# FanmingL/Recurrent-Offpolicy-RL

Hardware: AMD Instinct MI355X
Metric: env-steps/sec trained (higher is better)
Workload: dtype f32; 1 GPU; smamba_s32_c16_b2_nln SAC-REDQ update, B=64/GPU, T=1024, D=256 (configs[1]; N=8: configs[3]); row_length=1043, obs=17, act=6, critic=efc-8, global_rows=64, parallelism=dp1

## Files before the change

include/resel_hip.h:

```cpp
#ifndef RESEL_HIP_H
#define RESEL_HIP_H

#include <stddef.h>
#include <stdint.h>

#ifdef __cplusplus
extern "C" {
#endif

#define RESEL_OK 0
#define RESEL_EINVAL (-1)
#define RESEL_ELAUNCH (-2)

typedef void* resel_stream_t;

int resel_abi_version(void);
const char* resel_build_info(void);

enum {
    RESEL_PROF_SSCAN_FWD = 0, RESEL_PROF_SSCAN_BWD = 1, RESEL_PROF_ATTN_FWD = 2, RESEL_PROF_ATTN_DQ = 3, RESEL_PROF_ATTN_DKV = 4,
    RESEL_PROF_LINREC_REAL_FWD = 5, RESEL_PROF_LINREC_REAL_BWD = 6, RESEL_PROF_LINREC_COMPLEX_FWD = 7, RESEL_PROF_LINREC_COMPLEX_BWD = 8,
    RESEL_PROF_GRU_FWD = 9, RESEL_PROF_GRU_BWD = 10, RESEL_PROF_CONV_FWD = 11, RESEL_PROF_CONV_BWD = 12, RESEL_PROF_GEMM = 13,
    RESEL_PROF_SSCAN_FWD_LOCAL = 14, RESEL_PROF_SSCAN_BWD_LOCAL = 15,
    RESEL_PROF_NSLOTS = 16
// ... 10 lines not shown
                             const float* D, const float* delta_bias, const float* start,
                             float* out, int64_t ld_out, float* ckpt, float* last_state, void* workspace,
                             int B, int L, int Di, int N, int delta_softplus, int time_segments,
                             void* amax_out, unsigned amax_epoch, resel_stream_t stream);

size_t resel_selective_scan_bwd_workspace_bytes(int B, int L, int Di, int N, int time_segments);
int resel_selective_scan_bwd(const float* u, int64_t ld_u, const float* delta, int64_t ld_delta,
                             const float* z, int64_t ld_z, const float* A,
                             const float* Bm, int64_t ld_b, const float* Cm, int64_t ld_c,
                             const float* D, const float* delta_bias, const float* start,
                             const float* dout, int64_t ld_dout, const float* ckpt,
                             float* du, int64_t ld_du, float* ddelta, int64_t ld_ddelta, float* dz, int64_t ld_dz,
                             float* dBm, int64_t ld_db, float* dCm, int64_t ld_dc,
                             float* dA, float* dD, float* ddelta_bias, void* workspace,
                             int B, int L, int Di, int N, int delta_softplus, int time_segments,
                             void* amax_dz, void* amax_ddelta, unsigned amax_epoch, resel_stream_t stream);

int resel_causal_conv1d_fwd(const float* x, int64_t ld_x, const float* w, const float* bias, const float* mask,
                            float* y, int64_t ld_y, int B, int L, int Di, int K, int silu, void* amax_y, unsigned amax_epoch,
                            resel_stream_t stream);
size_t resel_causal_conv1d_bwd_workspace_bytes(int B, int L, int Di, int K);
int resel_causal_conv1d_bwd(const float* x, int64_t ld_x, const float* w, const float* bias, const float* mask,
                            const float* dy, int64_t ld_dy, float* dx, int64_t ld_dx, float* dw, float* dbias,
                            void* workspace, int B, int L, int Di, int K, int silu, void* amax_dx, unsigned amax_epoch,
                            resel_stream_t stream);
int resel_causal_conv1d_bwd2(const float* x, int64_t ld_x, const float* w, const float* bias, const float* mask,
                             const float* dy, int64_t ld_dy, const float* dy2, int64_t ld_dy2, float* dx, int64_t ld_dx,
                             float* dw, float* dbias, void* workspace, int B, int L, int Di, int K, int silu,
                             void* amax_dx, unsigned amax_epoch, resel_stream_t stream);

int resel_add_layernorm_fwd(const float* x, const float* residual, const float* w, const float* b,
                            float* y, float* res_out, float* stats, int M, int C, float eps, int rms, int act,
                            void* amax_y, unsigned amax_epoch, resel_stream_t stream);
size_t resel_add_layernorm_bwd_workspace_bytes(int M, int C);
int resel_add_layernorm_bwd(const float* dy, const float* dres_in, const float* res, const float* w, const float* b,
                            const float* stats, float* dx, float* dw, float* db, void* workspace,
                            int M, int C, int rms, int has_bias, int act, void* amax_dx, unsigned amax_epoch, resel_stream_t stream);

int resel_linrec_real_fwd(const float* v, const float* f, int64_t ld_u, const float* start, const float* h0, float* h,
                          int B, int L, int C, int fuse_act, void* amax_h, unsigned amax_epoch, resel_stream_t stream);
int resel_linrec_real_bwd(const float* v, const float* f, int64_t ld_u, const float* start, const float* h0, const float* h,
                          const float* dh, float* dv, float* df, int64_t ld_du, int B, int L, int C, int fuse_act,
                          void* amax_du, unsigned amax_epoch, resel_stream_t stream);
int resel_linrec_complex_fwd(const float* vr, const float* vi, int64_t ld_u, const float* lam_re, const float* lam_im,
                             const float* gamma, const float* start, const float* h0r, const float* h0i,
                             float* hr, float* hi, int B, int L, int C, void* amax_h, unsigned amax_epoch, resel_stream_t stream);
size_t resel_linrec_complex_bwd_workspace_bytes(int B, int L, int C);
int resel_linrec_complex_bwd(const float* vr, const float* vi, int64_t ld_u, const float* lam_re, const float* lam_im,
                             const float* gamma, const float* start, const float* h0r, const float* h0i,
                             const float* hr, const float* hi, const float* dhr, const float* dhi,
                             float* dvr, float* dvi, int64_t ld_du, float* dlam_re, float* dlam_im, float* dgamma,
                             void* workspace, int B, int L, int C, resel_stream_t stream);

int resel_lru_params_fwd(const float* params_log, float* out, int C, resel_stream_t stream);
int resel_lru_params_bwd(const float* params_log, const float* dout, float* dparams_log, int C, resel_stream_t stream);

size_t resel_gru_workspace_bytes(int B, int L, int H);
int resel_gru_seq_fwd(const float* gi, const float* w_hh, const float* b_hh, const float* h0,
                      float* h_all, float* gates, void* workspace, int B, int L, int H, resel_stream_t stream);
int resel_gru_seq_bwd(const float* w_hh, const float* h0, const float* h_all, const float* gates,
                      const float* dh_all, float* dgi, float* dgh, void* workspace,
                      int B, int L, int H, resel_stream_t stream);

size_t resel_attn_varlen_fwd_workspace_bytes(int S, int max_seqlen);
int resel_attn_varlen_fwd(const uint16_t* qkv, const int32_t* cu_seqlens, const float* slopes, uint16_t* out, float* lse,
                          void* workspace, int T, int S, int H, int hd, int max_seqlen, float scale,
                          float p_drop, uint64_t seed, uint64_t offset, resel_stream_t stream);
size_t resel_attn_varlen_bwd_workspace_bytes(int T, int S, int H, int hd, int max_seqlen);
int resel_attn_varlen_bwd(const uint16_t* qkv, const int32_t* cu_seqlens, const float* slopes, const uint16_t* out,
                          const float* lse, const uint16_t* dout, uint16_t* dqkv, void* workspace,
                          int T, int S, int H, int hd, int max_seqlen, float scale,
                          float p_drop, uint64_t seed, uint64_t offset, resel_stream_t stream);

int resel_dropout(const float* x, float* y, int64_t n, float p_drop, uint64_t seed, uint64_t offset, resel_stream_t stream);
int resel_dropout_offset_base(const void* base);
int resel_gelu_dropout_fwd(const float* x, float* y, int64_t n, float p_drop, uint64_t seed, uint64_t offset,
                           void* amax_y, unsigned amax_epoch, resel_stream_t stream);
int resel_gelu_dropout_bwd(const float* x, const float* dy, float* dx, int64_t n, float p_drop, uint64_t seed, uint64_t offset,
                           void* amax_dx, unsigned amax_epoch, resel_stream_t stream);

int resel_tanh_gaussian_fwd(const float* out2, const float* noise, float* action_mean, float* action_sample,
                            float* logp, int M, int A, resel_stream_t stream);
int resel_tanh_gaussian_bwd(const float* out2, const float* noise, const float* d_sample, const float* d_logp,
                            float* d_out2, int M, int A, resel_stream_t stream);

int resel_sac_target(const float* q, const int32_t* subset, int m, const float* next_logp, const float* log_alpha,
                     const float* reward, const float* done, const float* mask, float gamma, float* guard,
                     float* target, float* stats, void* workspace, int E, int M, resel_stream_t stream);
int resel_sac_target_phase(int phase, const float* q, const int32_t* subset, int m, const float* next_logp, const float* log_alpha,
                           const float* reward, const float* done, const float* mask, float gamma, float* guard,
                           float* target, float* stats, float* extrema, void* workspace, int E, int M, resel_stream_t stream);
int resel_sac_target_local(const float* q, const int32_t* subset, int m, const float* next_logp, const float* log_alpha,
                           const float* reward, const float* done, const float* mask, float gamma, const float* guard,
                           float* target, float* stats, float* extrema, void* workspace, int E, int M, resel_stream_t stream);
int resel_guard_apply_slots(const float* slots, int world, float* guard, resel_stream_t stream);
size_t resel_sac_target_workspace_bytes(int M);

size_t resel_masked_loss_workspace_bytes(void);
int resel_q_loss_fwd(const float* q, const float* y, const float* mask, float* out2, void* workspace, int E, int M, resel_stream_t stream);
int resel_q_loss_bwd(const float* q, const float* y, const float* mask, const float* g, float* dq, int E, int M, resel_stream_t stream);
int resel_actor_loss_fwd(const float* logp, const float* q, const float* mask, const float* log_alpha, float* out2, void* workspace,
                         int E, int M, int use_logp, int reduce_min, resel_stream_t stream);
int resel_actor_loss_bwd(const float* q, const float* mask, const float* log_alpha, const float* g, float* dlogp, float* dq,
                         int E, int M, int use_logp, int reduce_min, resel_stream_t stream);

int resel_soft_update(float* target, const float* online, float tau, int64_t n, resel_stream_t stream);
int resel_adamw_flat(float* p, const float* g, float* m, float* v, int64_t n, const int64_t* seg_end,
                     const float* seg_lr, const float* seg_wd, int nseg, float beta1, float beta2, float eps,
                     int step, const float* grad_scale, resel_stream_t stream);
int resel_adamw_flat_dev(float* p, const float* g, float* m, float* v, int64_t n, const int64_t* seg_end,
                         const float* seg_lr, const float* seg_wd, int nseg, float beta1, float beta2, float eps,
                         const float* bias_corrections, const float* grad_scale, resel_stream_t stream);
size_t resel_sumsq_workspace_bytes(int64_t n);
int resel_sumsq(const float* x, int64_t n, float* out, void* workspace, resel_stream_t stream);

int resel_bias_act_fwd(float* y, const float* bias, int64_t rows, int C, int64_t rows_per_seg, int act, resel_stream_t stream);
size_t resel_bias_act_bwd_workspace_bytes(int64_t rows, int C, int64_t rows_per_seg);
int resel_bias_act_bwd(const float* g, int64_t ldg, const float* a, int64_t lda, float* gy, float* dbias, void* workspace, int64_t rows, int C,
                       int64_t rows_per_seg, int act, void* amax_gy, unsigned amax_epoch, resel_stream_t stream);

int resel_ensemble_head_fwd(float* y, const float* b2, const float* w3, const float* b3, float* q, int64_t rows, int H,
                            int64_t rows_per_seg, resel_stream_t stream);
size_t resel_ensemble_head_bwd_workspace_bytes(int64_t rows, int H, int64_t rows_per_seg);
int resel_ensemble_head_bwd(const float* gq, const float* a, const float* w3, float* gy, float* db2, float* dw3, void* workspace,
                            int64_t rows, int H, int64_t rows_per_seg, void* amax_gy, unsigned amax_epoch, resel_stream_t stream);

size_t resel_gemm_f32_workspace_bytes(int M, int N, int K, int batch);
int resel_gemm_f32(const float* A, int64_t lda, int64_t strideA, int a_kcontig,
                   const float* B, int64_t ldb, int64_t strideB, int b_kcontig,
                   const float* bias, int64_t strideBias, int act,
                   float* C, int64_t ldc, int64_t strideC, void* workspace,
                   int M, int N, int K, int batch, int split, resel_stream_t stream);

int resel_gemm_f32x(const float* A, int64_t lda, int64_t strideA, int a_kcontig,
                    const float* B, int64_t ldb, int64_t strideB, int b_kcontig,
                    const float* bias, int64_t strideBias, int act,
                    float* C, int64_t ldc, int64_t strideC, void* workspace,
                    int M, int N, int K, int batch, int split, const float* amax_a, const float* amax_b,
                    void* amax_c, unsigned amax_epoch, resel_stream_t stream);
int resel_gemm_f32_fused_supported(int kind, int M, int N, int K, int64_t lda, int64_t ldb);
size_t resel_gemm_f32_fused_workspace_bytes(int M, int N, int K, int batch, int kind);
int resel_gemm_f32_dact(const float* A, int64_t lda, int64_t strideA, int a_kcontig,
                        const float* B, int64_t ldb, int64_t strideB, int b_kcontig,
                        const float* Y, int64_t ldy, int64_t strideY,
                        float* C, int64_t ldc, int64_t strideC, float* dbias, void* workspace,
                        int M, int N, int K, int batch, const float* amax_a, const float* amax_b,
                        void* amax_c, unsigned amax_epoch, resel_stream_t stream);
int resel_gemm_f32_head(const float* A, int64_t lda, int64_t strideA, int a_kcontig,
                        const float* B, int64_t ldb, int64_t strideB, int b_kcontig,
                        const float* bias, int64_t strideBias, const float* w3, int64_t strideW3, const float* b3,
                        float* C, int64_t ldc, int64_t strideC, float* q, void* workspace,
                        int M, int N, int K, int batch, const float* amax_a, const float* amax_b,
                        void* amax_c, unsigned amax_epoch, resel_stream_t stream);
int resel_place_blocks(float* out, int64_t ld_out, int rows, int cols, int nblk, const float* const* src, const int64_t* ld_src,
                       const int* r0, const int* nr, const int* c0, const int* nc, resel_stream_t stream);

int resel_amax_segments(const float* flat, const int64_t* begin, const int64_t* len, int nseg, void* handles, unsigned epoch,
                        resel_stream_t stream);
size_t resel_amax_state_bytes(void);
int resel_amax(const float* x, int64_t ld, int64_t stride, int rows, int cols, int batch, void* out, unsigned epoch, void* state,
               resel_stream_t stream);
int resel_amax_check(const float* x, int64_t ld, int64_t stride, int rows, int cols, int batch, const void* handle, int* err, int tag,
                     resel_stream_t stream);

size_t resel_gemm_bf16_workspace_bytes(int M, int N, int K);
int resel_gemm_bf16(const void* A, int64_t lda, int a_kcontig, int a_bf16, const void* B, int64_t ldb, int b_kcontig, int b_bf16,
                    const float* bias, void* C, int64_t ldc, int c_bf16, void* workspace, int M, int N, int K,
                    resel_stream_t stream);

size_t resel_colsum_bf16_workspace_bytes(int M, int N);
int resel_colsum_bf16(const uint16_t* x, int64_t ld, int M, int N, float* out, void* workspace, resel_stream_t stream);

int resel_gather_trajs(const float* buffer, int W, int64_t capacity, const int* segments, int nseg, int max_len, int skip, int rows, int Tp,
                       int c_mask, int c_start, int c_done, int c_timeout, const int* pre_pairs, int npairs,
                       float* out, resel_stream_t stream);

int resel_mamba_conv_step(const float* x, int64_t ldx, const float* state_in, int64_t ld_in, float* state_out, int64_t ld_out,
                          int64_t stride_d, int64_t stride_k, int W, const float* w, const float* bias, float* xc, int B, int Di,
                          int K, int act, resel_stream_t stream);
int resel_selective_state_update(const float* state_in, int64_t ld_in, float* state_out, int64_t ld_out, const float* xc,
                                 const float* x_db, int64_t ld_xdb, const float* w_dt, const float* dt_bias, const float* A_log,
                                 const float* D, const float* z, int64_t ldz, float* y, int B, int Di, int N, int R,
                                 resel_stream_t stream);
int resel_attn_decode(const uint16_t* qkv, int64_t ld_qkv, uint16_t* kv_cache, const int32_t* pos_dev, int pos_host,
                      const float* slopes, uint16_t* out, float scale, int B, int H, int head_dim, int max_seqlen,
                      resel_stream_t stream);

size_t resel_atb_workspace_bytes(int64_t K, int Wd, int Nd);
int resel_atb(const float* wide, int64_t ldw, int Wd, const float* narrow, int64_t ldn, int Nd, float* out, int transposed,
              void* workspace, int64_t K, resel_stream_t stream);

#ifdef __cplusplus
}
#endif
#endif
```

recurrent-offpolicy-rl_amd/csrc/bias_act.hip:

```cpp
#include "resel_common.h"

namespace {
using namespace resel;

constexpr int BWD_ROWS = 128;

__device__ __forceinline__ float elu_(float x) { return x > 0.f ? x : fast_exp(x) - 1.f; }

__global__ __launch_bounds__(256) void bias_act_fwd_kernel(float* __restrict__ y, const float* __restrict__ bias, int64_t rows,
                                                           int C, int64_t rows_per_seg, int act) {
    const int c4n = C / 4;
    const int64_t n4 = rows * c4n;
    for (int64_t i = (int64_t)blockIdx.x * blockDim.x + threadIdx.x; i < n4; i += (int64_t)gridDim.x * blockDim.x) {
        const int64_t r = i / c4n;
        const int c = (int)(i % c4n) * 4;
        float4 v = ld4(y + r * C + c);
        if (bias) {
            const float4 b = ld4(bias + (r / rows_per_seg) * C + c);
            v.x += b.x; v.y += b.y; v.z += b.z; v.w += b.w;
        }
        if (act == 1) { v.x = elu_(v.x); v.y = elu_(v.y); v.z = elu_(v.z); v.w = elu_(v.w); }
        st4(y + r * C + c, v);
    }
}

__global__ __launch_bounds__(256) void bias_act_bwd_kernel(const float* __restrict__ g, int64_t ldg, const float* __restrict__ a, int64_t lda,
                                                           float* __restrict__ gy, float* __restrict__ db_part,
                                                           int C, int64_t rows_per_seg, int act, int nrb, int brows, AmaxOut amax) {
    __shared__ __attribute__((aligned(16))) float s_red[4][256];
    const int cl = threadIdx.x & 63, rl = threadIdx.x >> 6;
    const int c = blockIdx.y * 256 + cl * 4;
    const int64_t seg = blockIdx.z;
    const int64_t r0 = (int64_t)blockIdx.x * brows;
    const int64_t r1 = r0 + brows < rows_per_seg ? r0 + brows : rows_per_seg;
    float4 acc = make_float4(0.f, 0.f, 0.f, 0.f);
    float gmax = 0.f;
    if (c < C) {
        for (int64_t r = r0 + rl; r < r1; r += 4) {
            const int64_t o = (seg * rows_per_seg + r) * C + c;
            float4 v = ld4(g + (seg * rows_per_seg + r) * ldg + c);
            if (act == 1) {
                const float4 av = ld4(a + (seg * rows_per_seg + r) * lda + c);
                v.x *= av.x > 0.f ? 1.f : av.x + 1.f; v.y *= av.y > 0.f ? 1.f : av.y + 1.f;
                v.z *= av.z > 0.f ? 1.f : av.z + 1.f; v.w *= av.w > 0.f ? 1.f : av.w + 1.f;
            }
            if (gy != nullptr) st4(gy + o, v);
            acc.x += v.x; acc.y += v.y; acc.z += v.z; acc.w += v.w;
            gmax = amax4(gmax, v);
        }
    }
    amax_publish_wave(gmax, amax);
    if (db_part == nullptr) return;
    st4(&s_red[rl][cl * 4], acc);
    __syncthreads();
    if (rl == 0 && c < C) {
        float4 t = ld4(&s_red[0][cl * 4]);
#pragma unroll
        for (int k = 1; k < 4; ++k) {
            const float4 q = ld4(&s_red[k][cl * 4]);
            t.x += q.x; t.y += q.y; t.z += q.z; t.w += q.w;
        }
        st4(db_part + ((seg * nrb + blockIdx.x) * (int64_t)C) + c, t);
    }
}

__global__ __launch_bounds__(256) void head_fwd_kernel(float* __restrict__ y, const float* __restrict__ b2, const float* __restrict__ w3,
                                                       const float* __restrict__ b3, float* __restrict__ q, int64_t rows, int H,
                                                       int64_t rows_per_seg) {
    const int lane = threadIdx.x & 63;
    const int64_t r = (int64_t)blockIdx.x * 4 + (threadIdx.x >> 6);
    if (r >= rows) return;
    const int64_t e = r / rows_per_seg;
    float acc = 0.f;
    for (int c = lane * 4; c < H; c += 256) {
        float4 v = ld4(y + r * H + c);
        const float4 b = ld4(b2 + e * H + c), w = ld4(w3 + e * H + c);
        v.x = elu_(v.x + b.x); v.y = elu_(v.y + b.y); v.z = elu_(v.z + b.z); v.w = elu_(v.w + b.w);
        st4(y + r * H + c, v);
        acc += v.x * w.x + v.y * w.y + v.z * w.z + v.w * w.w;
    }
    acc = wave_sum(acc);
    if (lane == 0) q[r] = acc + (b3 ? b3[e] : 0.f);
}

__global__ __launch_bounds__(256) void head_bwd_kernel(const float* __restrict__ gq, const float* __restrict__ a,
                                                       const float* __restrict__ w3, float* __restrict__ gy,
                                                       float* __restrict__ db_part, float* __restrict__ dw_part, int H,
                                                       int64_t rows_per_seg, int nrb, AmaxOut amax) {
    __shared__ __attribute__((aligned(16))) float s_red[2][4][256];
    const int cl = threadIdx.x & 63, rl = threadIdx.x >> 6;
    const int c = blockIdx.y * 256 + cl * 4;
    const int64_t seg = blockIdx.z;
    const int64_t r0 = (int64_t)blockIdx.x * BWD_ROWS;
    const int64_t r1 = r0 + BWD_ROWS < rows_per_seg ? r0 + BWD_ROWS : rows_per_seg;
    float4 accb = make_float4(0.f, 0.f, 0.f, 0.f), accw = accb;
    float gmax = 0.f;
    if (c < H) {
        const float4 w = ld4(w3 + seg * H + c);
        for (int64_t r = r0 + rl; r < r1; r += 4) {
            const int64_t row = seg * rows_per_seg + r;
            const float g = gq[row];
            const float4 av = ld4(a + row * H + c);
            float4 v;
            v.x = g * w.x * (av.x > 0.f ? 1.f : av.x + 1.f); v.y = g * w.y * (av.y > 0.f ? 1.f : av.y + 1.f);
            v.z = g * w.z * (av.z > 0.f ? 1.f : av.z + 1.f); v.w = g * w.w * (av.w > 0.f ? 1.f : av.w + 1.f);
            st4(gy + row * H + c, v);
            gmax = amax4(gmax, v);
            accb.x += v.x; accb.y += v.y; accb.z += v.z; accb.w += v.w;
            accw.x += g * av.x; accw.y += g * av.y; accw.z += g * av.z; accw.w += g * av.w;
        }
    }
    amax_publish_wave(gmax, amax);
    st4(&s_red[0][rl][cl * 4], accb);
    st4(&s_red[1][rl][cl * 4], accw);
    __syncthreads();
    if (rl < 2 && c < H) {
        float4 t = ld4(&s_red[rl][0][cl * 4]);
#pragma unroll
        for (int k = 1; k < 4; ++k) {
            const float4 qv = ld4(&s_red[rl][k][cl * 4]);
            t.x += qv.x; t.y += qv.y; t.z += qv.z; t.w += qv.w;
        }
        st4((rl == 0 ? db_part : dw_part) + ((seg * nrb + blockIdx.x) * (int64_t)H) + c, t);
    }
}

inline int row_blocks(int64_t rows_per_seg) { return (int)((rows_per_seg + BWD_ROWS - 1) / BWD_ROWS); }
inline int block_rows(int64_t, int, int64_t) { return BWD_ROWS; }
inline int row_blocks_of(int64_t rows_per_seg, int brows) { return (int)((rows_per_seg + brows - 1) / brows); }
inline bool shape_ok(int64_t rows, int C, int64_t rows_per_seg) {
    return rows > 0 && C > 0 && C % 4 == 0 && rows_per_seg > 0 && rows % rows_per_seg == 0;
}

}

extern "C" int resel_bias_act_fwd(float* y, const float* bias, int64_t rows, int C, int64_t rows_per_seg, int act,
                                  resel_stream_t stream) {
    if (!y || !shape_ok(rows, C, rows_per_seg) || act < 0 || act > 1 || !aligned16(y) || (bias && !aligned16(bias))) return RESEL_EINVAL;
    const int64_t n4 = rows * (C / 4);
    const int64_t want = (n4 + 255) / 256;
    const unsigned grid = (unsigned)(want < 256 * 32 ? want : 256 * 32);
    hipLaunchKernelGGL(bias_act_fwd_kernel, dim3(grid), dim3(256), 0, (hipStream_t)stream, y, bias, rows, C, rows_per_seg, act);
    return launch_status();
}

extern "C" size_t resel_bias_act_bwd_workspace_bytes(int64_t rows, int C, int64_t rows_per_seg) {
    if (!shape_ok(rows, C, rows_per_seg)) return 0;
    return (size_t)(rows / rows_per_seg) * row_blocks_of(rows_per_seg, block_rows(rows, C, rows_per_seg)) * C * sizeof(float);
}

extern "C" int resel_bias_act_bwd(const float* g, int64_t ldg, const float* a, int64_t lda, float* gy, float* dbias, void* workspace, int64_t rows, int C,
                                  int64_t rows_per_seg, int act, void* amax_gy, unsigned amax_epoch, resel_stream_t stream) {
    if (amax_gy && (reinterpret_cast<uintptr_t>(amax_gy) & 7u)) return RESEL_EINVAL;
    if (!g || !shape_ok(rows, C, rows_per_seg) || act < 0 || act > 1 || (act == 1 && (!a || !gy)) || (dbias && !workspace) || ldg < C || (ldg & 3))
        return RESEL_EINVAL;
    if (a && (lda < C || (lda & 3))) return RESEL_EINVAL;
    if (!aligned16(g) || (gy && !aligned16(gy)) || (a && !aligned16(a)) || (workspace && !aligned16(workspace))) return RESEL_EINVAL;
    const int brows = block_rows(rows, C, rows_per_seg);
    const int nseg = (int)(rows / rows_per_seg), nrb = row_blocks_of(rows_per_seg, brows);
    hipStream_t s = (hipStream_t)stream;
    float* part = dbias ? (float*)workspace : nullptr;
    hipLaunchKernelGGL(bias_act_bwd_kernel, dim3(nrb, (C + 255) / 256, nseg), dim3(256), 0, s, g, ldg, a, lda, gy, part, C, rows_per_seg, act, nrb, brows,
                       AmaxOut{(unsigned long long*)amax_gy, amax_epoch});
    if (dbias) launch_colsum(part, C, nrb, C, dbias, s, 1, 0, nseg);
    return launch_status();
}

extern "C" int resel_ensemble_head_fwd(float* y, const float* b2, const float* w3, const float* b3, float* q, int64_t rows, int H,
                                       int64_t rows_per_seg, resel_stream_t stream) {
    if (!y || !b2 || !w3 || !q || !shape_ok(rows, H, rows_per_seg) || !aligned16(y) || !aligned16(b2) || !aligned16(w3)) return RESEL_EINVAL;
    hipLaunchKernelGGL(head_fwd_kernel, dim3((unsigned)((rows + 3) / 4)), dim3(256), 0, (hipStream_t)stream, y, b2, w3, b3, q, rows, H,
                       rows_per_seg);
    return launch_status();
}

extern "C" size_t resel_ensemble_head_bwd_workspace_bytes(int64_t rows, int H, int64_t rows_per_seg) {
    return 2 * resel_bias_act_bwd_workspace_bytes(rows, H, rows_per_seg);
}

extern "C" int resel_ensemble_head_bwd(const float* gq, const float* a, const float* w3, float* gy, float* db2, float* dw3,
                                       void* workspace, int64_t rows, int H, int64_t rows_per_seg, void* amax_gy, unsigned amax_epoch,
                                       resel_stream_t stream) {
    if (amax_gy && (reinterpret_cast<uintptr_t>(amax_gy) & 7u)) return RESEL_EINVAL;
    if (!gq || !a || !w3 || !gy || !db2 || !dw3 || !workspace || !shape_ok(rows, H, rows_per_seg)) return RESEL_EINVAL;
    if (!aligned16(a) || !aligned16(w3) || !aligned16(gy) || !aligned16(workspace)) return RESEL_EINVAL;
    const int nseg = (int)(rows / rows_per_seg), nrb = row_blocks(rows_per_seg);
    hipStream_t s = (hipStream_t)stream;
    float* db_part = (float*)workspace;
    float* dw_part = db_part + (size_t)nseg * nrb * H;
    hipLaunchKernelGGL(head_bwd_kernel, dim3(nrb, (H + 255) / 256, nseg), dim3(256), 0, s, gq, a, w3, gy, db_part, dw_part, H, rows_per_seg, nrb,
                       AmaxOut{(unsigned long long*)amax_gy, amax_epoch});
    launch_colsum(db_part, H, nrb, H, db2, s, 1, 0, nseg);
    launch_colsum(dw_part, H, nrb, H, dw3, s, 1, 0, nseg);
    return launch_status();
}
```

recurrent-offpolicy-rl_amd/csrc/gemm_bf3.hip:

```cpp
#include "resel_common.h"
#include <algorithm>
#include <atomic>
#include <cstdlib>
#include <type_traits>

namespace {
using namespace resel;

typedef float f32x16 __attribute__((ext_vector_type(16)));
typedef __bf16 bf16x8 __attribute__((ext_vector_type(8)));
constexpr int BM = 256, BN = 128, BK = 32;
constexpr int NTH = 512;
constexpr int GRID = 256;
constexpr int TILE = BM * BN;
constexpr int ROWB = 64;
constexpr int PLA = BM * ROWB, PLB = BN * ROWB;
constexpr int STAGE = 3 * PLA + 3 * PLB;

struct Params {
    const float *A, *B, *bias;
    float *C, *slab;
    int64_t lda, ldb, ldc, sA, sB, sC, sBias;
    int M, N, K;
    int act;
    int mt, nt;
    int nfull, nsplit, nsl, kslice;
    const float *amaxA, *amaxB;
    AmaxOut amaxC;
    int ntst;
    const float* aux;
    int64_t ldaux, sAux;
    float* red;
    int redrows;
};

__device__ __forceinline__ float elu1(float x) { return x > 0.f ? x : fast_exp(x) - 1.f; }

__device__ __forceinline__ void tile_origin(const Params& p, int t, int& z, int& m0, int& n0) {
    const int ntile = p.mt * p.nt;
    z = t / ntile;
    const int tt = t - z * ntile;
    const int q = ntile / 8, r = ntile % 8, x = tt & 7, j = tt >> 3;
    const int bid = (x < r ? x * (q + 1) : r * (q + 1) + (x - r) * q) + j;
    m0 = (bid / p.nt) * BM;
    n0 = (bid % p.nt) * BN;
}
struct Item { int m0, n0, z, kbeg, kend, split; };
__device__ __forceinline__ Item decode(const Params& p, int it) {
    Item o;
    int t = it;
    o.kbeg = 0; o.kend = p.K; o.split = 0;
    if (it >= p.nfull) {
        const int idx = it - p.nfull, tr = idx / p.nsl, sl = idx - tr * p.nsl;
        t = p.nfull + tr;
        o.kbeg = sl * p.kslice; o.kend = min(p.K, o.kbeg + p.kslice); o.split = idx + 1;
    }
    tile_origin(p, t, o.z, o.m0, o.n0);
    return o;
}

__device__ __forceinline__ int plane_off(int row, int c) {
    const int q = row >> 2;
    return ((row ^ (q & 1)) << 6) + ((c ^ (q & 3)) << 4);
}

__device__ __forceinline__ uint32_t rne_pair(float lo, float hi) {
    typedef __bf16 bf16x2_t __attribute__((ext_vector_type(2)));
    typedef float f32x2_t __attribute__((ext_vector_type(2)));
    const f32x2_t v = {lo, hi};
    return __builtin_bit_cast(uint32_t, __builtin_convertvector(v, bf16x2_t));
}
struct P3 { uint2 p1, p2, p3; };
template <int NP>
__device__ __forceinline__ P3 split4(const float4& v) {
#ifdef BF3_AB_NOSPLIT
    return P3{make_uint2(__float_as_uint(v.x), __float_as_uint(v.y)), make_uint2(__float_as_uint(v.z), __float_as_uint(v.w)),
              make_uint2(__float_as_uint(v.x), __float_as_uint(v.w))};
#endif
    const float x[4] = {v.x, v.y, v.z, v.w};
    uint32_t w1[2], w2[2], w3[2] = {0u, 0u};
#pragma unroll
    for (int q = 0; q < 2; ++q) {
        const uint32_t u0 = __float_as_uint(x[2 * q]), u1 = __float_as_uint(x[2 * q + 1]);
        w1[q] = __builtin_amdgcn_perm(u1, u0, 0x07060302u);
        const float r0 = x[2 * q] - __uint_as_float(u0 & 0xffff0000u), r1 = x[2 * q + 1] - __uint_as_float(u1 & 0xffff0000u);
        if (NP == 2) {
            w2[q] = rne_pair(r0, r1);
        } else {
            const uint32_t v0 = __float_as_uint(r0), v1 = __float_as_uint(r1);
            w2[q] = __builtin_amdgcn_perm(v1, v0, 0x07060302u);
            const float s0 = r0 - __uint_as_float(v0 & 0xffff0000u), s1 = r1 - __uint_as_float(v1 & 0xffff0000u);
            w3[q] = __builtin_amdgcn_perm(__float_as_uint(s1), __float_as_uint(s0), 0x07060302u);
        }
    }
    return P3{make_uint2(w1[0], w1[1]), make_uint2(w2[0], w2[1]), make_uint2(w3[0], w3[1])};
}
struct P3h { uint32_t p1, p2, p3; };
template <int NP>
__device__ __forceinline__ P3h split2(float x0, float x1) {
    const uint32_t u0 = __float_as_uint(x0), u1 = __float_as_uint(x1);
    P3h o;
    o.p1 = __builtin_amdgcn_perm(u1, u0, 0x07060302u);
    const float r0 = x0 - __uint_as_float(u0 & 0xffff0000u), r1 = x1 - __uint_as_float(u1 & 0xffff0000u);
    if (NP == 2) {
        o.p2 = rne_pair(r0, r1);
        o.p3 = 0u;
        return o;
    }
    const uint32_t v0 = __float_as_uint(r0), v1 = __float_as_uint(r1);
    o.p2 = __builtin_amdgcn_perm(v1, v0, 0x07060302u);
    const float s0 = r0 - __uint_as_float(v0 & 0xffff0000u), s1 = r1 - __uint_as_float(v1 & 0xffff0000u);
    o.p3 = __builtin_amdgcn_perm(__float_as_uint(s1), __float_as_uint(s0), 0x07060302u);
    return o;
}

typedef _Float16 f16x2_t __attribute__((ext_vector_type(2)));
typedef float f32x2_t __attribute__((ext_vector_type(2)));
template <bool WIDE>
__device__ __forceinline__ void split_pair_f16(float x0, float x1, f32x2_t sc, uint32_t& p1, uint32_t& p2, uint32_t& p3) {
#ifdef BF3_AB_NOSPLIT
    p1 = __float_as_uint(x0); p2 = __float_as_uint(x1); p3 = __float_as_uint(x0) ^ __float_as_uint(sc.x);
    return;
#endif
    const f32x2_t xs = {x0 * sc.x, x1 * sc.x};
    const f16x2_t h = __builtin_convertvector(xs, f16x2_t);
    p1 = __builtin_bit_cast(uint32_t, h);
    if (WIDE) {
        const f32x2_t r = {__builtin_fmaf((float)h.x, -2048.f, x0 * sc.y), __builtin_fmaf((float)h.y, -2048.f, x1 * sc.y)};
        p2 = __builtin_bit_cast(uint32_t, __builtin_convertvector(r, f16x2_t));
        p3 = 0u;
    } else {
        const f32x2_t r = {xs.x - (float)h.x, xs.y - (float)h.y};
        p2 = __builtin_bit_cast(uint32_t, __builtin_convertvector(r, f16x2_t));
        p3 = 0u;
    }
}
template <bool WIDE>
__device__ __forceinline__ P3 split4_f16(const float4& v, f32x2_t sc) {
    P3 o;
    split_pair_f16<WIDE>(v.x, v.y, sc, o.p1.x, o.p2.x, o.p3.x);
    split_pair_f16<WIDE>(v.z, v.w, sc, o.p1.y, o.p2.y, o.p3.y);
    return o;
}
template <bool WIDE>
__device__ __forceinline__ P3h split2_f16(float x0, float x1, f32x2_t sc) {
    P3h o;
    split_pair_f16<WIDE>(x0, x1, sc, o.p1, o.p2, o.p3);
    return o;
}
__device__ __forceinline__ float f16_scale(float amax) {
    const int f = (int)((__float_as_uint(amax) >> 23) & 0xffu);
    const int e = min(max(268 - f, 1), 240);
    return __uint_as_float((uint32_t)e << 23);
}

template <bool KC, int ROWS>
struct Src {
    static constexpr int NPC = ROWS / 64;
    static constexpr bool is_kc = KC;
    static constexpr int NR = KC ? NPC : (ROWS == 256 ? 4 : 2);
    const char* base;
    const char* base0;
    uint32_t off[NR];
    uint32_t loff[KC ? NPC : 4];
    int64_t step;
    int rl0, rlim, ld4, kofs4;
    int kofs;
    float4 r[NR];
    __device__ __forceinline__ void init(const float* P, int64_t ld, int rows, int r0, int k0, int tid) {
        if (KC) {
            kofs = 4 * (tid & 7);
            base = (const char*)(P + (int64_t)r0 * ld + k0);
            base0 = (const char*)(P + (int64_t)r0 * ld);
#pragma unroll
            for (int i = 0; i < NPC; ++i) {
                const int rl = (tid >> 3) + 64 * i;
                off[i] = (uint32_t)(((r0 + rl < rows ? rl : 0) * ld + kofs) * 4);
            }
            step = BK * 4;
            rl0 = tid >> 3;
            rlim = min(rows - 1 - r0, ROWS - 1);
            ld4 = (int)(ld * 4);
            kofs4 = kofs * 4;
        } else {
            const int g = ROWS == 256 ? (tid & 7) + 8 * (tid >> 6) : (tid & 7) + 8 * (tid >> 7);
            kofs = ROWS == 256 ? 4 * ((tid >> 3) & 7) : 2 * ((tid >> 3) & 15);
// ... 270 lines not shown
            for (int b = 0; b < 2; ++b)
#pragma unroll
                for (int e = 0; e < 16; ++e) acc[a][b][e] = zero;
        float bv[2] = {0.f, 0.f};

        for (int c_k0 = cur.kbeg; c_k0 < cur.kend; c_k0 += BK) {
            const int so = cur_st * STAGE, sn = (cur_st ^ 1) * STAGE;
            const bool fast = p_live && p_k0 + BK <= p_kend;
            if (c_k0 + BK >= cur.kend && p.bias && !cur.split) {
#pragma unroll
                for (int b = 0; b < 2; ++b) {
                    const int n = cur.n0 + wn + 32 * b + li;
                    bv[b] = p.bias[(int64_t)cur.z * p.sBias + (n < p.N ? n : 0)];
                }
            }
            BF3_FENCE();
            read_a<NP>(f1, fa[1] + so); read_b<NPB>(f1, fb[1] + so);
            mfma_small<SPLIT>(acc, f0);
            stage_store(cur_st ^ 1);
            if (F16) mfma_lead_f16(acc, f0); else mfma_lead(acc, f0);
            sa.load_sched(fast);
            sb.load_sched(fast);
            mfma_small<SPLIT>(acc, f1);
            if (SPLIT == 3 || SPLIT == 2) {
#pragma unroll
                for (int i = 0; i < 12; ++i) {
                    __builtin_amdgcn_sched_group_barrier(0x008, 1, 0);
                    if (i < 2 * (NP + NPB)) __builtin_amdgcn_sched_group_barrier(0x100, 1, 0);
                    __builtin_amdgcn_sched_group_barrier(0x002, 8, 0);
                    __builtin_amdgcn_sched_group_barrier(0x200, 1, 0);
                    if (i >= 4) __builtin_amdgcn_sched_group_barrier(0x020, 1, 0);
                }
            } else {
                constexpr int NMA = SPLIT == 9 ? 60 : 36;
#pragma unroll
                for (int i = 0; i < NMA; ++i) {
                    __builtin_amdgcn_sched_group_barrier(0x008, 1, 0);
                    if (i < 12) __builtin_amdgcn_sched_group_barrier(0x100, 1, 0);
                    __builtin_amdgcn_sched_group_barrier(0x002, SPLIT == 9 ? 3 : 5, 0);
                    if (i >= 4 && i < 4 + 18) __builtin_amdgcn_sched_group_barrier(0x200, 1, 0);
                    if (i >= NMA - 8) __builtin_amdgcn_sched_group_barrier(0x020, 1, 0);
                }
            }
            BF3_FENCE();
#ifdef BF3_AB_NOBAR
            asm volatile("s_waitcnt lgkmcnt(0)" ::: "memory");
#else
            asm volatile("s_waitcnt lgkmcnt(0)\n\ts_barrier" ::: "memory");
#endif
            BF3_FENCE();
            read_a<NP>(f0, fa[0] + sn); read_b<NPB>(f0, fb[0] + sn);
            if (F16) mfma_lead_f16(acc, f1); else mfma_lead(acc, f1);
#pragma unroll
            for (int i = 0; i < 12; ++i) {
                __builtin_amdgcn_sched_group_barrier(0x008, 1, 0);
                if (i < 2 * (NP + NPB)) __builtin_amdgcn_sched_group_barrier(0x100, 1, 0);
            }
            BF3_FENCE();
            if (fast) {
                p_k0 += BK;
                if (p_k0 >= p_kend) {
                    p_item += G;
                    if (p_item < total) p_open(); else p_live = false;
                }
            } else {
                produce();
            }
            BF3_FENCE();
            cur_st ^= 1;
        }
        if (F16) {
#pragma unroll
            for (int a = 0; a < 2; ++a)
#pragma unroll
                for (int b = 0; b < 2; ++b)
#pragma unroll
                    for (int e = 0; e < 16; ++e) acc[a][b][e] *= unscale;
        }
#ifdef BF3_AB_NOEPI
        if (lane == 0) p.C[(int64_t)cur.m0 * p.ldc + cur.n0 + w] = acc[0][0][0] + acc[0][1][1] + acc[1][0][2] + acc[1][1][3];
        continue;
#endif
        if (cur.split) {
            float* o = p.slab + (int64_t)(cur.split - 1) * TILE + (wm + 4 * lh) * BN + wn + li;
#pragma unroll
            for (int a = 0; a < 2; ++a)
#pragma unroll
                for (int b = 0; b < 2; ++b)
#pragma unroll
                    for (int e = 0; e < 16; ++e) o[(32 * a + (e & 3) + 8 * (e >> 2)) * BN + 32 * b] = acc[a][b][e];
        } else {
            float* C = p.C + (int64_t)cur.z * p.sC;
            const bool full_m = cur.m0 + BM <= p.M;
#pragma unroll
            for (int b = 0; b < 2; ++b) {
                const int n = cur.n0 + wn + 32 * b + li;
                if (n >= p.N) continue;
#pragma unroll
                for (int a = 0; a < 2; ++a) {
                    float v[16];
#pragma unroll
                    for (int e = 0; e < 16; ++e) v[e] = acc[a][b][e] + bv[b];
                    if (p.act == 1) {
#pragma unroll
                        for (int e = 0; e < 16; ++e) v[e] = elu1(v[e]);
                    }
                    if (p.act == 3) {
#pragma unroll
                        for (int e = 0; e < 16; ++e) v[e] = softplus_nb(v[e]);
                    }
                    const int mb = cur.m0 + wm + 32 * a + 4 * lh;
                    float* crow = C + (int64_t)mb * p.ldc + n;
                    if (p.act == 2) {
#pragma unroll
                        for (int e = 0; e < 16; ++e) {
                            const int dm = (e & 3) + 8 * (e >> 2);
                            if (mb + dm < p.M) v[e] += crow[(int64_t)dm * p.ldc];
                        }
                    }
                    if (full_m) {
#pragma unroll
                        for (int e = 0; e < 16; ++e) crow[(int64_t)((e & 3) + 8 * (e >> 2)) * p.ldc] = v[e];
                    } else {
#pragma unroll
                        for (int e = 0; e < 16; ++e) {
                            const int dm = (e & 3) + 8 * (e >> 2);
                            if (mb + dm < p.M) crow[(int64_t)dm * p.ldc] = v[e];
                        }
                    }
                    if (p.amaxC.slot) {
#pragma unroll
                        for (int e = 0; e < 16; e += 2) cmax = fmaxf(cmax, fmaxf(__builtin_fabsf(v[e]), __builtin_fabsf(v[e + 1])));
                    }
                }
            }
        }
    }
    amax_publish_wave(cmax, p.amaxC);
#ifdef BF3_AB_CLOCK
    if (tid == 0) {
        g_bf3_clock[2 * blockIdx.x] = __builtin_amdgcn_s_memtime() - ck_t0;
        g_bf3_clock[2 * blockIdx.x + 1] = __builtin_amdgcn_s_memrealtime() - ck_r0;
    }
#endif
}

constexpr int NTH_WS = 512;
constexpr int WS_LDS = 2 * STAGE;
#define WS_BARRIER() asm volatile("s_waitcnt lgkmcnt(0)\n\ts_barrier" ::: "memory")

template <bool AKC, bool BKC, int SPLIT, int EPI = 0>
__global__ __launch_bounds__(NTH_WS, 1) void gemm_ws_kernel(Params p) {
    extern __shared__ __attribute__((aligned(16))) char lds[];
    constexpr bool F16 = SPLIT == 2;
    constexpr int NP = (SPLIT == 3 || SPLIT == 2) ? 2 : 3;
    constexpr int NPB = (SPLIT == 3 || SPLIT == 2) ? 2 : 3;
    const int tid = threadIdx.x;
    const int total = p.nfull + p.nsplit * p.nsl;
    const int G = gridDim.x;
    if ((int)blockIdx.x >= total) return;
    float sa_ = 1.f, sb_ = 1.f;
    if (F16) { sa_ = f16_scale(amax_read(p.amaxA)); sb_ = f16_scale(amax_read(p.amaxB)); }
    asm volatile("" :: "v"(sa_), "v"(sb_));

    if (__builtin_amdgcn_readfirstlane(tid) >= 256) {
        const int pt = tid - 256;
        const f32x2_t scA = {sa_, 2048.f * sa_}, scB = {sb_, 2048.f * sb_};
        typedef Src<AKC, BM> SA;
        typedef Src<BKC, BN> SB;
        SA a0, a1;
        SB b0, b1;
        a0.init_lds(pt); a1.init_lds(pt + 256);
        b0.init_lds(pt); b1.init_lds(pt + 256);
        typedef float f32x4a __attribute__((ext_vector_type(4)));
        f32x4a ra[2][2][SA::NR], rb[2][2][SB::NR];
        int nsteps = 0;
        for (int it = blockIdx.x; it < total; it += G) {
            const Item i = decode(p, it);
            nsteps += (i.kend - i.kbeg + BK - 1) / BK;
        }
        int p_item = blockIdx.x, p_k0 = 0, p_kend = 0;
        bool p_live = true;
        auto p_open = [&]() {
            const Item it = decode(p, p_item);
            const float* Ab = p.A + (int64_t)it.z * p.sA;
            const float* Bb = p.B + (int64_t)it.z * p.sB;
            a0.init(Ab, p.lda, p.M, it.m0, it.kbeg, pt); a1.init(Ab, p.lda, p.M, it.m0, it.kbeg, pt + 256);
            b0.init(Bb, p.ldb, p.N, it.n0, it.kbeg, pt); b1.init(Bb, p.ldb, p.N, it.n0, it.kbeg, pt + 256);
            p_k0 = it.kbeg; p_kend = it.kend;
        };
        auto advance = [&]() {
            a0.base += a0.step; a1.base += a1.step; b0.base += b0.step; b1.base += b1.step;
            p_k0 += BK;
            if (p_k0 >= p_kend) {
                p_item += G;
                if (p_item < total) p_open(); else p_live = false;
            }
        };
        auto aload = [&](f32x4a& r, const char* base, uint32_t off) {
#ifdef BF3_AB_NOLOAD
            asm volatile("" : "+v"(r) : "v"(off), "s"(base) : "memory");
#else
            asm volatile("global_load_dwordx4 %0, %1, %2" : "=v"(r) : "v"(off), "s"(base) : "memory");
#endif
        };
        auto issue_set = [&](auto SET) {
            constexpr int S = decltype(SET)::value;
            auto all = [&](auto& src, auto& regs) {
                typedef std::remove_reference_t<decltype(src)> ST;
#pragma unroll
                for (int i = 0; i < ST::NR; ++i) {
                    if constexpr (ST::is_kc) aload(regs[i], src.base, src.piece_off(i));
                    else aload(regs[i], src.base, src.off[i]);
                }
            };
            all(a0, ra[S][0]); all(a1, ra[S][1]); all(b0, rb[S][0]); all(b1, rb[S][1]);
            advance();
        };
        constexpr int FA = F16 ? 1 : 0, FB = F16 ? 2 : 0;
        auto recycle = [&](auto SET, auto MODEC) {
            constexpr int S = decltype(SET)::value;
            constexpr int MODE = decltype(MODEC)::value;
            constexpr bool LOAD = MODE == 0;
            uint32_t st_off = S * STAGE;
            asm volatile("" : "+s"(st_off));
            char* st = lds + st_off;
            auto one = [&](auto& src, auto& regs, char* pl, f32x2_t sc, auto PLc, auto NPc, auto Fc) {
                constexpr int PL = decltype(PLc)::value, NPP = decltype(NPc)::value, FF = decltype(Fc)::value;
                typedef std::remove_reference_t<decltype(src)> ST;
                if constexpr (ST::is_kc) {
#pragma unroll
                    for (int i = 0; i < ST::NR; ++i) {
                        if (LOAD) asm volatile("s_waitcnt vmcnt(23)" : "+v"(regs[i]) :: "memory");
                        const float4 v = make_float4(regs[i].x, regs[i].y, regs[i].z, regs[i].w);
                        const P3 sp = FF == 1 ? split4_f16<true>(v, sc) : FF == 2 ? split4_f16<false>(v, sc) : split4<NPP>(v);
                        char* d = pl + src.loff[0] + 4096 * i;
                        *reinterpret_cast<uint2*>(d) = sp.p1;
                        *reinterpret_cast<uint2*>(d + PL) = sp.p2;
                        if (NPP == 3) *reinterpret_cast<uint2*>(d + 2 * PL) = sp.p3;
                        if (MODE != 1) aload(regs[i], src.base, src.piece_off(i));
                    }
                } else {
                    float4 t[ST::NR];
                    if constexpr (ST::NR == 4) { if (LOAD) asm volatile("s_waitcnt vmcnt(20)" : "+v"(regs[0]), "+v"(regs[1]), "+v"(regs[2]), "+v"(regs[3]) :: "memory"); }
                    else { if (LOAD) asm volatile("s_waitcnt vmcnt(22)" : "+v"(regs[0]), "+v"(regs[1]) :: "memory"); }
#pragma unroll
                    for (int i = 0; i < ST::NR; ++i) t[i] = make_float4(regs[i].x, regs[i].y, regs[i].z, regs[i].w);
                    src.template store_from<PL, NPP, FF>(t, pl, sc);
                    if (MODE != 1) {
#pragma unroll
                        for (int i = 0; i < ST::NR; ++i) aload(regs[i], src.base, src.off[i]);
                    }
                }
            };
            using IA = std::integral_constant<int, PLA>;
            using IB = std::integral_constant<int, PLB>;
            one(a0, ra[S][0], st, scA, IA{}, std::integral_constant<int, NP>{}, std::integral_constant<int, FA>{});
            one(a1, ra[S][1], st, scA, IA{}, std::integral_constant<int, NP>{}, std::integral_constant<int, FA>{});
            one(b0, rb[S][0], st + 3 * PLA, scB, IB{}, std::integral_constant<int, NPB>{}, std::integral_constant<int, FB>{});
            one(b1, rb[S][1], st + 3 * PLA, scB, IB{}, std::integral_constant<int, NPB>{}, std::integral_constant<int, FB>{});
            if (MODE != 1) advance();
        };
        auto landed = [&]() {
#pragma unroll
            for (int q = 0; q < 2; ++q)
#pragma unroll
                for (int v = 0; v < 2; ++v) {
#pragma unroll
                    for (int i = 0; i < SA::NR; ++i) asm volatile("s_waitcnt vmcnt(0)" : "+v"(ra[q][v][i]) :: "memory");
#pragma unroll
                    for (int i = 0; i < SB::NR; ++i) asm volatile("s_waitcnt vmcnt(0)" : "+v"(rb[q][v][i]) :: "memory");
                }
        };
        using S0 = std::integral_constant<int, 0>;
        using S1 = std::integral_constant<int, 1>;
        using M0 = std::integral_constant<int, 0>;
        using M1 = std::integral_constant<int, 1>;
        using M2 = std::integral_constant<int, 2>;
        p_open();
        issue_set(S0{});
        if (nsteps > 1) issue_set(S1{});
        int j = 0;
        for (; j + 3 < nsteps; j += 2) {
            recycle(S0{}, M0{});
            WS_BARRIER();
            recycle(S1{}, M0{});
            WS_BARRIER();
        }
        landed();
        for (; j < nsteps; ++j) {
            const bool more = j + 2 < nsteps;
            if (j & 1) { if (more) recycle(S1{}, M2{}); else recycle(S1{}, M1{}); }
            else { if (more) recycle(S0{}, M2{}); else recycle(S0{}, M1{}); }
            if (more) landed();
            WS_BARRIER();
        }
        WS_BARRIER();
        return;
    }

    static_assert(SPLIT == 2, "the 4 + 4 wave form exists for mode 2");
    const float unscale = (1.f / sa_) * (1.f / sb_);
    const int lane = tid & 63, w = tid >> 6;
    const int wm = (w >> 1) * 128, wn = (w & 1) * 64;
    const int li = lane & 31, lh = lane >> 5;
    const char* fa[2];
    const char* fb[2];
#pragma unroll
    for (int s = 0; s < 2; ++s) {
        fa[s] = lds + wm * ROWB + plane_off(li, 2 * s + lh);
        fb[s] = lds + 3 * PLA + wn * ROWB + plane_off(li, 2 * s + lh);
    }
    struct F4 { f16x8 a[2][4], b[2][2]; };
    auto rd = [&](F4& f, const char* pa, const char* pb) {
#pragma unroll
        for (int pi = 0; pi < 2; ++pi) {
#pragma unroll
            for (int t = 0; t < 4; ++t) f.a[pi][t] = *reinterpret_cast<const f16x8*>(pa + pi * PLA + t * 32 * ROWB);
#pragma unroll
            for (int t = 0; t < 2; ++t) f.b[pi][t] = *reinterpret_cast<const f16x8*>(pb + pi * PLB + t * 32 * ROWB);
        }
    };
    f32x16 acc[4][2];
    auto mm = [&](const F4& f) {
        const f16x8 k = {(_Float16)0.00048828125f, (_Float16)0.00048828125f, (_Float16)0.00048828125f, (_Float16)0.00048828125f,
                         (_Float16)0.00048828125f, (_Float16)0.00048828125f, (_Float16)0.00048828125f, (_Float16)0.00048828125f};
        const f16x8 bs0 = f.b[0][0] * k, bs1 = f.b[0][1] * k;
#ifdef BF3_AB_NOMFMA
#pragma unroll
        for (int a = 0; a < 4; ++a) asm volatile("" :: "v"(f.a[0][a]), "v"(f.a[1][a]), "v"(bs0), "v"(bs1), "v"(f.b[0][0]), "v"(f.b[0][1]), "v"(f.b[1][0]), "v"(f.b[1][1]));
        return;
#endif
#pragma unroll
        for (int a = 0; a < 4; ++a) {
            acc[a][0] = __builtin_amdgcn_mfma_f32_32x32x16_f16(f.a[1][a], bs0, acc[a][0], 0, 0, 0);
            acc[a][1] = __builtin_amdgcn_mfma_f32_32x32x16_f16(f.a[1][a], bs1, acc[a][1], 0, 0, 0);
        }
#pragma unroll
        for (int q = 1; q >= 0; --q)
#pragma unroll
            for (int a = 0; a < 4; ++a) {
                acc[a][0] = __builtin_amdgcn_mfma_f32_32x32x16_f16(f.a[0][a], f.b[q][0], acc[a][0], 0, 0, 0);
                acc[a][1] = __builtin_amdgcn_mfma_f32_32x32x16_f16(f.a[0][a], f.b[q][1], acc[a][1], 0, 0, 0);
            }
    };
    float cmax = 0.f;
    F4 f0, f1;
    WS_BARRIER();
    rd(f0, fa[0], fb[0]);
    int cur_st = 0;
    constexpr bool DEFER_F0 = EPI == 4;
    for (int c_item = blockIdx.x; c_item < total; c_item += G) {
        const Item cur = decode(p, c_item);
        if (DEFER_F0 && c_item != (int)blockIdx.x) rd(f0, fa[0] + cur_st * STAGE, fb[0] + cur_st * STAGE);
        float zero = 0.f;
        asm volatile("" : "+v"(zero));
#pragma unroll
        for (int a = 0; a < 4; ++a)
#pragma unroll
            for (int b = 0; b < 2; ++b)
#pragma unroll
                for (int e = 0; e < 16; ++e) acc[a][b][e] = zero;
        float bv[2] = {0.f, 0.f};
        for (int c_k0 = cur.kbeg; c_k0 < cur.kend; c_k0 += BK) {
            const int so = cur_st * STAGE, sn = (cur_st ^ 1) * STAGE;
            if (c_k0 + BK >= cur.kend && p.bias && !cur.split) {
#pragma unroll
                for (int b = 0; b < 2; ++b) {
                    const int n = cur.n0 + wn + 32 * b + li;
                    bv[b] = p.bias[(int64_t)cur.z * p.sBias + (n < p.N ? n : 0)];
                }
            }
            BF3_FENCE();
            rd(f1, fa[1] + so, fb[1] + so);
            mm(f0);
#pragma unroll
            for (int i = 0; i < 12; ++i) {
                __builtin_amdgcn_sched_group_barrier(0x008, 1, 0);
                __builtin_amdgcn_sched_group_barrier(0x100, 1, 0);
            }
            BF3_FENCE();
            WS_BARRIER();
            BF3_FENCE();
            if (!(DEFER_F0 && c_k0 + BK >= cur.kend)) rd(f0, fa[0] + sn, fb[0] + sn);
            mm(f1);
#pragma unroll
            for (int i = 0; i < 12; ++i) {
                __builtin_amdgcn_sched_group_barrier(0x008, 1, 0);
                __builtin_amdgcn_sched_group_barrier(0x100, 1, 0);
            }
            BF3_FENCE();
            cur_st ^= 1;
        }
#ifdef BF3_AB_NOEPI
        if (lane == 0) p.C[(int64_t)cur.m0 * p.ldc + cur.n0 + w] = acc[0][0][0] + acc[1][1][1] + acc[2][0][2] + acc[3][1][3];
        continue;
#endif
#pragma unroll
        for (int a = 0; a < 4; ++a)
#pragma unroll
            for (int b = 0; b < 2; ++b)
#pragma unroll
                for (int e = 0; e < 16; ++e) acc[a][b][e] *= unscale;
        if (cur.split) {
            float* o = p.slab + (int64_t)(cur.split - 1) * TILE + (wm + 4 * lh) * BN + wn + li;
#pragma unroll
            for (int a = 0; a < 4; ++a)
#pragma unroll
                for (int b = 0; b < 2; ++b)
#pragma unroll
                    for (int e = 0; e < 16; ++e) o[(32 * a + (e & 3) + 8 * (e >> 2)) * BN + 32 * b] = acc[a][b][e];
            continue;
        }
        if constexpr (EPI == 0) {
            float* C = p.C + (int64_t)cur.z * p.sC;
            const bool full_m = cur.m0 + BM <= p.M;
            if (full_m && cur.n0 + BN <= p.N && p.act != 2) {
                char* sc = lds + (w >> 1) * STAGE + 2 * PLA + (w & 1) * 5120;
                float* wr = reinterpret_cast<float*>(sc) + (4 * lh) * 40 + li;
                const float4* rdp = reinterpret_cast<const float4*>(sc + (lane >> 3) * 160 + (lane & 7) * 16);
#pragma unroll
                for (int b = 0; b < 2; ++b) {
#pragma unroll
                    for (int a = 0; a < 4; ++a) {
                        float v[16];
#pragma unroll
                        for (int e = 0; e < 16; ++e) v[e] = acc[a][b][e] + bv[b];
                        if (p.act == 1) {
#pragma unroll
                            for (int e = 0; e < 16; ++e) v[e] = elu1(v[e]);
                        }
                        if (p.act == 3) {
#pragma unroll
                            for (int e = 0; e < 16; ++e) v[e] = softplus_nb(v[e]);
                        }
                        if (p.amaxC.slot) {
#pragma unroll
                            for (int e = 0; e < 16; e += 2) cmax = fmaxf(cmax, fmaxf(__builtin_fabsf(v[e]), __builtin_fabsf(v[e + 1])));
                        }
#pragma unroll
                        for (int e = 0; e < 16; ++e) wr[((e & 3) + 8 * (e >> 2)) * 40] = v[e];
                        float* q = C + (int64_t)(cur.m0 + wm + 32 * a + (lane >> 3)) * p.ldc + cur.n0 + wn + 32 * b + 4 * (lane & 7);
#pragma unroll
                        for (int g = 0; g < 4; ++g) {
                            const float4 t = rdp[g * 8 * 10];
                            if (p.ntst) {
                                typedef float f4v __attribute__((ext_vector_type(4)));
                                __builtin_nontemporal_store(f4v{t.x, t.y, t.z, t.w}, reinterpret_cast<f4v*>(q + (int64_t)(8 * g) * p.ldc));
                            } else {
                                *reinterpret_cast<float4*>(q + (int64_t)(8 * g) * p.ldc) = t;
                            }
                        }
                    }
                }
                continue;
            }
#pragma unroll
            for (int b = 0; b < 2; ++b) {
                const int n = cur.n0 + wn + 32 * b + li;
                if (n >= p.N) continue;
#pragma unroll
                for (int a = 0; a < 4; ++a) {
                    float v[16];
#pragma unroll
                    for (int e = 0; e < 16; ++e) v[e] = acc[a][b][e] + bv[b];
                    if (p.act == 1) {
#pragma unroll
                        for (int e = 0; e < 16; ++e) v[e] = elu1(v[e]);
                    }
                    if (p.act == 3) {
#pragma unroll
                        for (int e = 0; e < 16; ++e) v[e] = softplus_nb(v[e]);
                    }
                    const int mb = cur.m0 + wm + 32 * a + 4 * lh;
                    float* crow = C + (int64_t)mb * p.ldc + n;
                    if (p.act == 2) {
#pragma unroll
                        for (int e = 0; e < 16; ++e) {
                            const int dm = (e & 3) + 8 * (e >> 2);
                            if (mb + dm < p.M) v[e] += crow[(int64_t)dm * p.ldc];
                        }
                    }
                    if (full_m) {
#pragma unroll
                        for (int e = 0; e < 16; ++e) crow[(int64_t)((e & 3) + 8 * (e >> 2)) * p.ldc] = v[e];
                    } else {
#pragma unroll
                        for (int e = 0; e < 16; ++e) {
                            const int dm = (e & 3) + 8 * (e >> 2);
                            if (mb + dm < p.M) crow[(int64_t)dm * p.ldc] = v[e];
                        }
                    }
                    if (p.amaxC.slot) {
#pragma unroll
                        for (int e = 0; e < 16; e += 2) cmax = fmaxf(cmax, fmaxf(__builtin_fabsf(v[e]), __builtin_fabsf(v[e + 1])));
                    }
                }
            }
        } else {
            float* C = p.C + (int64_t)cur.z * p.sC;
            const bool full_m = cur.m0 + BM <= p.M;
            constexpr bool DACT = EPI == 4, HEAD = EPI == 5;
            const int act = EPI ? (HEAD ? 1 : 0) : p.act;
            if constexpr (DACT) {
                constexpr int PF = 3;
                const int lane = (int)__builtin_amdgcn_mbcnt_hi(~0u, __builtin_amdgcn_mbcnt_lo(~0u, 0u));
                const int li = lane & 31, lh = lane >> 5;
                const int w = __builtin_amdgcn_readfirstlane(threadIdx.x >> 6);
                const int wm = (w >> 1) * 128, wn = (w & 1) * 64;
                typedef float f32x4a __attribute__((ext_vector_type(4)));
                f32x4a yv[8][4];
                char* sc = lds + (w >> 1) * STAGE + 2 * PLA + (w & 1) * 5120;
                float* wr = reinterpret_cast<float*>(sc) + (4 * lh) * 40 + li;
                float4* rdp = reinterpret_cast<float4*>(sc + (lane >> 3) * 160 + (lane & 7) * 16);
                const uint32_t ylane = (uint32_t)(((lane >> 3) * (int)p.ldaux + 4 * (lane & 7)) * 4);
                const float* ybase = p.aux + (int64_t)cur.z * p.sAux + (int64_t)(cur.m0 + wm) * p.ldaux + cur.n0 + wn;
                auto yld = [](f32x4a& r, uint32_t off, const float* base) {
                    asm volatile("global_load_dwordx4 %0, %1, %2" : "=v"(r) : "v"(off), "s"(base) : "memory");
                };
                auto ywait = [](f32x4a& r0, f32x4a& r1, f32x4a& r2, f32x4a& r3, auto NC) {
                    asm volatile("s_waitcnt vmcnt(%4)" : "+v"(r0), "+v"(r1), "+v"(r2), "+v"(r3) : "n"(decltype(NC)::value) : "memory");
                };
                auto yload = [&](auto TC) {
                    constexpr int t = decltype(TC)::value;
                    if constexpr (t < 8) {
                        const float* yb = ybase + (int64_t)(32 * (t >> 1)) * p.ldaux + 32 * (t & 1);
#pragma unroll
                        for (int g = 0; g < 4; ++g) yld(yv[t][g], ylane, yb + (int64_t)(8 * g) * p.ldaux);
                    }
                };
                float cs[2] = {0.f, 0.f}, cmx = 0.f;
                auto mul = [&](auto TC) {
                    constexpr int t = decltype(TC)::value;
                    constexpr int a = t >> 1, b = t & 1;
                    yload(std::integral_constant<int, t + PF>{});
                    ywait(yv[t][0], yv[t][1], yv[t][2], yv[t][3], std::integral_constant<int, 4 * ((t + PF < 7 ? t + PF : 7) - t)>{});
#pragma unroll
                    for (int g = 0; g < 4; ++g) rdp[g * 8 * 10] = make_float4(yv[t][g].x, yv[t][g].y, yv[t][g].z, yv[t][g].w);
#pragma unroll
                    for (int e = 0; e < 16; ++e) {
                        const float y = wr[((e & 3) + 8 * (e >> 2)) * 40];
                        const float v = acc[a][b][e] * (y > 0.f ? 1.f : y + 1.f);
                        acc[a][b][e] = v;
                        cs[b] += v;
                        cmx = fmaxf(cmx, __builtin_fabsf(v));
                    }
                };
                yload(std::integral_constant<int, 0>{}); yload(std::integral_constant<int, 1>{}); yload(std::integral_constant<int, 2>{});
                static_assert(PF == 3, "the prologue issues PF tiles");
                mul(std::integral_constant<int, 0>{}); mul(std::integral_constant<int, 1>{}); mul(std::integral_constant<int, 2>{});
                mul(std::integral_constant<int, 3>{}); mul(std::integral_constant<int, 4>{}); mul(std::integral_constant<int, 5>{});
                mul(std::integral_constant<int, 6>{}); mul(std::integral_constant<int, 7>{});
                if (p.red) {
#pragma unroll
                    for (int b = 0; b < 2; ++b) {
                        const float c = cs[b] + __shfl_xor(cs[b], 32, 64);
                        if (lh == 0) p.red[((int64_t)cur.z * p.redrows + 2 * (cur.m0 / BM) + (w >> 1)) * p.N + cur.n0 + wn + 32 * b + li] = c;
                    }
                }
                amax_publish_wave(cmx, p.amaxC);
#pragma unroll
                for (int b = 0; b < 2; ++b) {
#pragma unroll
                    for (int a = 0; a < 4; ++a) {
#pragma unroll
                        for (int e = 0; e < 16; ++e) wr[((e & 3) + 8 * (e >> 2)) * 40] = acc[a][b][e];
                        float* q = C + (int64_t)(cur.m0 + wm + 32 * a + (lane >> 3)) * p.ldc + cur.n0 + wn + 32 * b + 4 * (lane & 7);
#pragma unroll
                        for (int g = 0; g < 4; ++g) {
                            const float4 t = rdp[g * 8 * 10];
                            typedef float f4v __attribute__((ext_vector_type(4)));
                            __builtin_nontemporal_store(f4v{t.x, t.y, t.z, t.w}, reinterpret_cast<f4v*>(q + (int64_t)(8 * g) * p.ldc));
                        }
                    }
                }
                continue;
            }
            if (full_m && cur.n0 + BN <= p.N && act != 2) {
                char* sc = lds + (w >> 1) * STAGE + 2 * PLA + (w & 1) * 5120;
                float* wr = reinterpret_cast<float*>(sc) + (4 * lh) * 40 + li;
                const float4* rdp = reinterpret_cast<const float4*>(sc + (lane >> 3) * 160 + (lane & 7) * 16);
                auto tile = [&](int a, int b, const float4 (&yv)[4], float4& cs, const float4& w3, float (&qr)[4]) {
                    float v[16];
#pragma unroll
                    for (int e = 0; e < 16; ++e) v[e] = acc[a][b][e] + bv[b];
                    if (act == 1) {
#pragma unroll
                        for (int e = 0; e < 16; ++e) v[e] = elu1(v[e]);
                    }
                    if (act == 3) {
#pragma unroll
                        for (int e = 0; e < 16; ++e) v[e] = softplus_nb(v[e]);
                    }
                    if (p.amaxC.slot && !DACT) {
#pragma unroll
                        for (int e = 0; e < 16; e += 2) cmax = fmaxf(cmax, fmaxf(__builtin_fabsf(v[e]), __builtin_fabsf(v[e + 1])));
                    }
#pragma unroll
                    for (int e = 0; e < 16; ++e) wr[((e & 3) + 8 * (e >> 2)) * 40] = v[e];
                    float* q = C + (int64_t)(cur.m0 + wm + 32 * a + (lane >> 3)) * p.ldc + cur.n0 + wn + 32 * b + 4 * (lane & 7);
#pragma unroll
                    for (int g = 0; g < 4; ++g) {
                        float4 t = rdp[g * 8 * 10];
                        if (DACT) {
                            t.x *= yv[g].x > 0.f ? 1.f : yv[g].x + 1.f; t.y *= yv[g].y > 0.f ? 1.f : yv[g].y + 1.f;
                            t.z *= yv[g].z > 0.f ? 1.f : yv[g].z + 1.f; t.w *= yv[g].w > 0.f ? 1.f : yv[g].w + 1.f;
                            cs.x += t.x; cs.y += t.y; cs.z += t.z; cs.w += t.w;
                            if (p.amaxC.slot) cmax = amax4(cmax, t);
                        }
                        if (HEAD) qr[g] += (t.x * w3.x + t.y * w3.y) + (t.z * w3.z + t.w * w3.w);
                        if (p.ntst) {
                            typedef float f4v __attribute__((ext_vector_type(4)));
                            __builtin_nontemporal_store(f4v{t.x, t.y, t.z, t.w}, reinterpret_cast<f4v*>(q + (int64_t)(8 * g) * p.ldc));
                        } else {
                            *reinterpret_cast<float4*>(q + (int64_t)(8 * g) * p.ldc) = t;
                        }
                    }
                };
                if constexpr (EPI == 0) {
                    const float4 z4 = make_float4(0.f, 0.f, 0.f, 0.f);
                    const float4 nov[4] = {z4, z4, z4, z4};
                    float4 ncs = z4;
                    float nq[4] = {0.f, 0.f, 0.f, 0.f};
#pragma unroll
                    for (int b = 0; b < 2; ++b)
#pragma unroll
                        for (int a = 0; a < 4; ++a) tile(a, b, nov, ncs, z4, nq);
                } else {
                    const float4 z4 = make_float4(0.f, 0.f, 0.f, 0.f);
                    {
                        const float4 nov[4] = {z4, z4, z4, z4};
                        float4 ncs = z4, w3[2];
#pragma unroll
                        for (int b = 0; b < 2; ++b) w3[b] = ld4(p.aux + (int64_t)cur.z * p.sAux + cur.n0 + wn + 32 * b + 4 * (lane & 7));
#pragma unroll
                        for (int a = 0; a < 4; ++a) {
                            float qr[4] = {0.f, 0.f, 0.f, 0.f};
#pragma unroll
                            for (int b = 0; b < 2; ++b) tile(a, b, nov, ncs, w3[b], qr);
                            float* qp = p.red + ((int64_t)cur.z * 2 * p.nt + 2 * (cur.n0 / BN) + (w & 1)) * p.M + cur.m0 + wm + 32 * a + (lane >> 3);
#pragma unroll
                            for (int g = 0; g < 4; ++g) {
                                float r = qr[g];
                                r += __shfl_xor(r, 1, 64); r += __shfl_xor(r, 2, 64); r += __shfl_xor(r, 4, 64);
                                if ((lane & 7) == 0) qp[8 * g] = r;
                            }
                        }
                    }
                }
                continue;
            }
            float cs1[2] = {0.f, 0.f};
#pragma unroll
            for (int a = 0; a < 4; ++a) {
                float qe[16];
                if (HEAD) {
#pragma unroll
                    for (int e = 0; e < 16; ++e) qe[e] = 0.f;
                }
                const int mb = cur.m0 + wm + 32 * a + 4 * lh;
#pragma unroll
                for (int b = 0; b < 2; ++b) {
                    const int n = cur.n0 + wn + 32 * b + li;
                    if (n >= p.N) continue;
                    float v[16];
#pragma unroll
                    for (int e = 0; e < 16; ++e) v[e] = acc[a][b][e] + bv[b];
                    if (act == 1) {
#pragma unroll
                        for (int e = 0; e < 16; ++e) v[e] = elu1(v[e]);
                    }
                    if (act == 3) {
#pragma unroll
                        for (int e = 0; e < 16; ++e) v[e] = softplus_nb(v[e]);
                    }
                    if (DACT) {
                        const float* yrow = p.aux + (int64_t)cur.z * p.sAux + (int64_t)mb * p.ldaux + n;
#pragma unroll
                        for (int e = 0; e < 16; ++e) {
                            const int dm = (e & 3) + 8 * (e >> 2);
                            float y = 0.f;
                            if (mb + dm < p.M) y = yrow[(int64_t)dm * p.ldaux]; else v[e] = 0.f;
                            v[e] *= y > 0.f ? 1.f : y + 1.f;
                            cs1[b] += v[e];
                        }
                    }
                    if (HEAD) {
                        const float w3 = p.aux[(int64_t)cur.z * p.sAux + n];
#pragma unroll
                        for (int e = 0; e < 16; ++e) qe[e] += v[e] * w3;
                    }
                    float* crow = C + (int64_t)mb * p.ldc + n;
                    if (act == 2) {
#pragma unroll
                        for (int e = 0; e < 16; ++e) {
                            const int dm = (e & 3) + 8 * (e >> 2);
                            if (mb + dm < p.M) v[e] += crow[(int64_t)dm * p.ldc];
                        }
                    }
                    if (full_m) {
// ... 231 lines not shown
                        typedef float f4v __attribute__((ext_vector_type(4)));
                        __builtin_nontemporal_store(f4v{t.x, t.y, t.z, t.w}, reinterpret_cast<f4v*>(q + (int64_t)(8 * g) * p.ldc));
                    }
                }
            }
        } else {
#pragma unroll
            for (int b = 0; b < 2; ++b) {
                const int n = n0 + wn + 32 * b + li;
                if (n >= p.N) continue;
#pragma unroll
                for (int a = 0; a < 4; ++a) {
                    float v[16];
#pragma unroll
                    for (int e = 0; e < 16; ++e) v[e] = acc[a][b][e] + bv[b];
                    if (p.act == 1) {
#pragma unroll
                        for (int e = 0; e < 16; ++e) v[e] = elu1(v[e]);
                    }
                    if (p.act == 3) {
#pragma unroll
                        for (int e = 0; e < 16; ++e) v[e] = softplus_nb(v[e]);
                    }
                    const int mb = m0 + wm + 32 * a + 4 * lh;
                    float* crow = C + (int64_t)mb * p.ldc + n;
#pragma unroll
                    for (int e = 0; e < 16; ++e) {
                        const int dm = (e & 3) + 8 * (e >> 2);
                        if (mb + dm < p.M) crow[(int64_t)dm * p.ldc] = v[e];
                    }
                    if (p.amaxC.slot) {
#pragma unroll
                        for (int e = 0; e < 16; e += 2) cmax = fmaxf(cmax, fmaxf(__builtin_fabsf(v[e]), __builtin_fabsf(v[e + 1])));
                    }
                }
            }
        }
        __syncthreads();
    }
    amax_publish_wave(cmax, p.amaxC);
}

__global__ __launch_bounds__(256) void gemm_bf3_fixup_kernel(Params p) {
    __shared__ float4 part[3][64];
    const int tr = blockIdx.y, q = threadIdx.y;
    const int e = blockIdx.x * 64 + threadIdx.x, ml = e >> 5, nl = 4 * (e & 31);
    const float* s = p.slab + (int64_t)tr * p.nsl * TILE + ml * BN + nl;
    float4 v = make_float4(0.f, 0.f, 0.f, 0.f);
    int i = q;
    for (; i + 12 < p.nsl; i += 16) {
        const float4 u0 = ld4(s + (int64_t)i * TILE), u1 = ld4(s + (int64_t)(i + 4) * TILE);
        const float4 u2 = ld4(s + (int64_t)(i + 8) * TILE), u3 = ld4(s + (int64_t)(i + 12) * TILE);
        v.x = (((v.x + u0.x) + u1.x) + u2.x) + u3.x; v.y = (((v.y + u0.y) + u1.y) + u2.y) + u3.y;
        v.z = (((v.z + u0.z) + u1.z) + u2.z) + u3.z; v.w = (((v.w + u0.w) + u1.w) + u2.w) + u3.w;
    }
    for (; i < p.nsl; i += 4) {
        const float4 u = ld4(s + (int64_t)i * TILE);
        v.x += u.x; v.y += u.y; v.z += u.z; v.w += u.w;
    }
    if (q) part[q - 1][threadIdx.x] = v;
    __syncthreads();
    if (q) return;
    const float4 g1 = part[0][threadIdx.x], g2 = part[1][threadIdx.x], g3 = part[2][threadIdx.x];
    float o[4] = {(v.x + g1.x) + (g2.x + g3.x), (v.y + g1.y) + (g2.y + g3.y), (v.z + g1.z) + (g2.z + g3.z), (v.w + g1.w) + (g2.w + g3.w)};
    int z, m0, n0;
    tile_origin(p, p.nfull + tr, z, m0, n0);
    const int m = m0 + ml, n = n0 + nl;
    float cmax = 0.f;
    if (m < p.M && n < p.N) {
        float* c = p.C + (int64_t)z * p.sC + (int64_t)m * p.ldc + n;
#pragma unroll
        for (int j = 0; j < 4; ++j) {
            if (n + j >= p.N) break;
            float x = o[j] + (p.bias ? p.bias[(int64_t)z * p.sBias + n + j] : 0.f);
            if (p.act == 1) x = elu1(x);
            if (p.act == 3) x = softplus_nb(x);
            if (p.act == 2) x += c[j];
            c[j] = x;
            cmax = fmaxf(cmax, __builtin_fabsf(x));
        }
    }
    amax_publish_wave(cmax, p.amaxC);
}

struct Plan { int nfull, nsplit, nsl, kslice; };
constexpr int g_split_min_ksteps = 4;
inline Plan make_plan(int M, int N, int K, int batch) {
    const long nbt = (long)((M + BM - 1) / BM) * ((N + BN - 1) / BN) * batch;
    const int ksteps = (K + BK - 1) / BK;
    Plan pl{(int)nbt, 0, 1, ksteps * BK};
    const int r = (int)(nbt % GRID);
    if (r == 0 || r > GRID / 2 || ksteps < g_split_min_ksteps) return pl;
    int s = std::min(GRID / r, ksteps / 2);
    const int per = (ksteps + s - 1) / s;
    s = (ksteps + per - 1) / per;
    if (s < 2) return pl;
    pl.nfull = (int)(nbt - r); pl.nsplit = r; pl.nsl = s; pl.kslice = per * BK;
    return pl;
}

template <bool AKC, bool BKC, int SP>
int launch_one(const Params& p, dim3 grid, hipStream_t s) {
    static std::atomic<bool> attr_set[64];
    int dev = 0;
    if (hipGetDevice(&dev) != hipSuccess || dev < 0 || dev >= 64) return RESEL_ELAUNCH;
    if (!attr_set[dev].load(std::memory_order_acquire)) {
        if (hipFuncSetAttribute((const void*)gemm_bf3_kernel<AKC, BKC, SP>, hipFuncAttributeMaxDynamicSharedMemorySize, 2 * STAGE) != hipSuccess)
            return RESEL_ELAUNCH;
        attr_set[dev].store(true, std::memory_order_release);
    }
    launch_timed(RESEL_PROF_GEMM, gemm_bf3_kernel<AKC, BKC, SP>, grid, dim3(NTH), (size_t)(2 * STAGE), s, p);
    return RESEL_OK;
}

template <bool AKC, bool BKC, int SP, int EPI = 0>
int launch_ws(const Params& p, dim3 grid, hipStream_t s) {
    static std::atomic<bool> attr_set[64];
    int dev = 0;
    if (hipGetDevice(&dev) != hipSuccess || dev < 0 || dev >= 64) return RESEL_ELAUNCH;
    if (!attr_set[dev].load(std::memory_order_acquire)) {
        if (hipFuncSetAttribute((const void*)gemm_ws_kernel<AKC, BKC, SP, EPI>, hipFuncAttributeMaxDynamicSharedMemorySize, WS_LDS) != hipSuccess)
            return RESEL_ELAUNCH;
        attr_set[dev].store(true, std::memory_order_release);
    }
    launch_timed(RESEL_PROF_GEMM, gemm_ws_kernel<AKC, BKC, SP, EPI>, grid, dim3(NTH_WS), (size_t)WS_LDS, s, p);
    return RESEL_OK;
}

constexpr int g_nt = 1;
int g_edition = [] { const char* e = getenv("RESEL_GEMM_EDITION"); return e ? atoi(e) : 3; }();

}

#ifdef BF3_AB_CLOCK
extern "C" int resel_bf3_debug_clock(unsigned long long* host_out) {
    return (int)hipMemcpyFromSymbol(host_out, HIP_SYMBOL(g_bf3_clock), sizeof(unsigned long long) * 2 * GRID);
}
#endif

namespace resel {

size_t gemm_bf3_workspace_bytes(int M, int N, int K, int batch) {
    const Plan pl = make_plan(M, N, K, batch);
    return (size_t)pl.nsplit * pl.nsl * TILE * sizeof(float);
}

bool gemm_bf3_fused_ok(int M, int N, int K, int64_t lda, int64_t ldb) {
    return g_edition == 3 && M > 128 && N >= 4 && K >= BK && K % BK == 0 && lda < (1 << 22) && ldb < (1 << 22);
}

int gemm_bf3_launch(const float* A, int64_t lda, int64_t strideA, int a_kcontig, const float* B, int64_t ldb, int64_t strideB, int b_kcontig,
                    const float* bias, int64_t strideBias, int act, float* C, int64_t ldc, int64_t strideC, void* workspace,
                    int M, int N, int K, int batch, int split, hipStream_t s, const float* amaxA, const float* amaxB,
                    unsigned long long* amax_c, unsigned amax_epoch, const float* aux, int64_t ldaux, int64_t strideAux, float* red, int redrows) {
    if (split == 2 && (!amaxA || !amaxB)) return RESEL_EINVAL;
    Plan pl = make_plan(M, N, K, batch);
    if (act >= 4) {
        if (split != 2 || !gemm_bf3_fused_ok(M, N, K, lda, ldb) || !aux) return RESEL_EINVAL;
        if (act == 4 && (M % BM || N % BN)) return RESEL_EINVAL;
        const long nbt = (long)((M + BM - 1) / BM) * ((N + BN - 1) / BN) * batch;
        pl = Plan{(int)nbt, 0, 1, (K + BK - 1) / BK * BK};
    }
    if (pl.nsplit && (!workspace || !aligned16(workspace))) return RESEL_EINVAL;
    Params p{A, B, bias, C, (float*)workspace, lda, ldb, ldc, strideA, strideB, strideC, strideBias, M, N, K, act,
             (M + BM - 1) / BM, (N + BN - 1) / BN, pl.nfull, pl.nsplit, pl.nsl, pl.kslice, amaxA, amaxB, AmaxOut{amax_c, amax_epoch}, g_nt,
             aux, ldaux, strideAux, red, redrows};
    const int64_t total = (int64_t)pl.nfull + (int64_t)pl.nsplit * pl.nsl;
    dim3 grid((unsigned)std::min<int64_t>(total, GRID));
    int rc;
#define BF3_LAUNCH(SP) \
    do { if (a_kcontig && b_kcontig) rc = launch_one<true, true, SP>(p, grid, s); \
         else if (a_kcontig) rc = launch_one<true, false, SP>(p, grid, s); \
         else if (b_kcontig) rc = launch_one<false, true, SP>(p, grid, s); \
         else rc = launch_one<false, false, SP>(p, grid, s); } while (0)
#define WS_LAUNCH(SP) \
    do { if (a_kcontig && b_kcontig) rc = launch_ws<true, true, SP>(p, grid, s); \
         else if (a_kcontig) rc = launch_ws<true, false, SP>(p, grid, s); \
         else if (b_kcontig) rc = launch_ws<false, true, SP>(p, grid, s); \
         else rc = launch_ws<false, false, SP>(p, grid, s); } while (0)
    const bool ws = g_edition >= 3 && split == 2 && K % BK == 0 && pl.kslice % BK == 0 && lda < (1 << 22) && ldb < (1 << 22);
    if (g_edition == 4 && split == 2 && act != 2 && act < 4 && a_kcontig && batch == 1 && K % BK == 0 && K >= 2 * BK && M >= 2048 && N >= 192 &&
        ((N + BN8 - 1) / BN8 * BN8 - N) < 128 && lda < (1 << 22) && ldb < (1 << 22)) {
        Params q = p;
        q.nt = (N + BN8 - 1) / BN8;
        q.nfull = q.mt * q.nt;
        q.nsplit = 0;
        dim3 g8((unsigned)std::min<int64_t>(q.nfull, GRID));
        static std::atomic<bool> attr8[2][64];
        int dev = 0;
        if (hipGetDevice(&dev) != hipSuccess || dev < 0 || dev >= 64) return RESEL_ELAUNCH;
        if (!attr8[b_kcontig ? 1 : 0][dev].load(std::memory_order_acquire)) {
            const void* fn = b_kcontig ? (const void*)gemm_w8_kernel<true> : (const void*)gemm_w8_kernel<false>;
            if (hipFuncSetAttribute(fn, hipFuncAttributeMaxDynamicSharedMemorySize, W8_LDS) != hipSuccess) return RESEL_ELAUNCH;
            attr8[b_kcontig ? 1 : 0][dev].store(true, std::memory_order_release);
        }
        if (b_kcontig) launch_timed(RESEL_PROF_GEMM, gemm_w8_kernel<true>, g8, dim3(512), (size_t)W8_LDS, s, q);
        else launch_timed(RESEL_PROF_GEMM, gemm_w8_kernel<false>, g8, dim3(512), (size_t)W8_LDS, s, q);
        return launch_status();
    }
    if (act >= 4) {
        if (!a_kcontig) return RESEL_EINVAL;
        if (act == 4) rc = b_kcontig ? launch_ws<true, true, 2, 4>(p, grid, s) : launch_ws<true, false, 2, 4>(p, grid, s);
        else rc = b_kcontig ? launch_ws<true, true, 2, 5>(p, grid, s) : launch_ws<true, false, 2, 5>(p, grid, s);
    } else if (ws) WS_LAUNCH(2);
    else if (split == 3) BF3_LAUNCH(3); else if (split == 2) BF3_LAUNCH(2); else BF3_LAUNCH(6);
#undef WS_LAUNCH
#undef BF3_LAUNCH
    if (rc != RESEL_OK) return rc;
    if (pl.nsplit) hipLaunchKernelGGL(gemm_bf3_fixup_kernel, dim3(TILE / 4 / 64, pl.nsplit), dim3(64, 4), 0, s, p);
#ifdef BF3_AB_FIXUP2
    if (pl.nsplit && act != 2) hipLaunchKernelGGL(gemm_bf3_fixup_kernel, dim3(TILE / 4 / 64, pl.nsplit), dim3(64, 4), 0, s, p);
#endif
    return launch_status();
}

}
```

recurrent-offpolicy-rl_amd/csrc/gemm_f32.hip:

```cpp
#include "resel_common.h"
#include <algorithm>
#include <cstdlib>

namespace resel {
size_t gemm_bf3_workspace_bytes(int M, int N, int K, int batch);
int gemm_bf3_launch(const float* A, int64_t lda, int64_t strideA, int a_kcontig, const float* B, int64_t ldb, int64_t strideB, int b_kcontig,
                    const float* bias, int64_t strideBias, int act, float* C, int64_t ldc, int64_t strideC, void* workspace,
                    int M, int N, int K, int batch, int split, hipStream_t s, const float* amaxA, const float* amaxB,
                    unsigned long long* amax_c, unsigned amax_epoch, const float* aux = nullptr, int64_t ldaux = 0, int64_t strideAux = 0,
                    float* red = nullptr, int redrows = 0);
bool gemm_bf3_fused_ok(int M, int N, int K, int64_t lda, int64_t ldb);
}

namespace {
using namespace resel;

typedef float f32x16 __attribute__((ext_vector_type(16)));
constexpr int BM = 128, BN = 128, BK = 32, NG = BK / 8;
constexpr int LDK = BK + 4;
constexpr int GRID = 512;
constexpr int TILE = BM * BN;

struct GemmParams {
    const float *A, *B, *bias;
    float *C, *slab;
    int64_t lda, ldb, ldc, sA, sB, sC, sBias;
    int M, N, K;
    int act;
    int mt, nt;
    int nfull;
    int nsplit, nsl, kslice;
    AmaxOut amaxC;
};

__device__ __forceinline__ float elu1(float x) { return x > 0.f ? x : fast_exp(x) - 1.f; }

__device__ __forceinline__ void tile_origin(const GemmParams& p, int t, int& z, int& m0, int& n0) {
    const int ntile = p.mt * p.nt;
    z = t / ntile;
    const int tt = t - z * ntile;
    const int q = ntile / 8, r = ntile % 8, x = tt & 7, j = tt >> 3;
    const int bid = (x < r ? x * (q + 1) : r * (q + 1) + (x - r) * q) + j;
    m0 = (bid / p.nt) * BM;
    n0 = (bid % p.nt) * BN;
}

struct Item { int m0, n0, z, kbeg, kend, split; };
__device__ __forceinline__ Item decode(const GemmParams& p, int it) {
    Item o;
    int t = it;
    o.kbeg = 0; o.kend = p.K; o.split = 0;
    if (it >= p.nfull) {
        const int idx = it - p.nfull, tr = idx / p.nsl, sl = idx - tr * p.nsl;
        t = p.nfull + tr;
        o.kbeg = sl * p.kslice; o.kend = min(p.K, o.kbeg + p.kslice); o.split = idx + 1;
    }
    tile_origin(p, t, o.z, o.m0, o.n0);
    return o;
}

template <bool KC>
struct Src {
    const char* base;
    const char* base0;
    uint32_t off[4];
    int64_t step;
    int kofs;
    __device__ __forceinline__ void init(const float* P, int64_t ld, int rows, int r0, int k0, int tid) {
        kofs = 4 * (tid & 7);
        if (KC) {
            base = (const char*)(P + (int64_t)r0 * ld + k0);
            base0 = (const char*)(P + (int64_t)r0 * ld);
#pragma unroll
            for (int i = 0; i < 4; ++i) {
                const int rl = (tid >> 3) + 32 * i;
                off[i] = (uint32_t)(((r0 + rl < rows ? rl : 0) * ld + kofs) * 4);
            }
            step = BK * 4;
        } else {
            base = (const char*)(P + (int64_t)k0 * ld + r0);
            base0 = (const char*)(P + r0);
            const int rl = 4 * (tid >> 3);
#pragma unroll
            for (int j = 0; j < 4; ++j) off[j] = (uint32_t)(((kofs + j) * ld + (r0 + rl < rows ? rl : 0)) * 4);
            step = (int64_t)BK * ld * 4;
        }
    }
    __device__ __forceinline__ void load_sched(float4 (&r)[4], bool full) {
        const char* b = full ? base : base0;
#pragma unroll
        for (int i = 0; i < 4; ++i) r[i] = *reinterpret_cast<const float4*>(b + off[i]);
        if (full) base += step;
    }
    __device__ __forceinline__ void load(float4 (&r)[4], int k0, int kend) {
        if (k0 + BK <= kend) {
#pragma unroll
            for (int i = 0; i < 4; ++i) r[i] = *reinterpret_cast<const float4*>(base + off[i]);
        } else {
#pragma unroll
            for (int i = 0; i < 4; ++i) {
                r[i] = make_float4(0.f, 0.f, 0.f, 0.f);
                if (k0 + kofs + (KC ? 0 : i) < kend) r[i] = *reinterpret_cast<const float4*>(base + off[i]);
            }
        }
        base += step;
    }
};
template <bool KC>
__device__ __forceinline__ void tile_store(float* __restrict__ S, int tid, const float4 (&r)[4]) {
    if (KC) {
#pragma unroll
        for (int i = 0; i < 4; ++i) st4(S + ((tid >> 3) + 32 * i) * LDK + 4 * (tid & 7), r[i]);
    } else {
        float* q = S + (4 * (tid >> 3)) * LDK + 4 * (tid & 7);
        st4(q, make_float4(r[0].x, r[1].x, r[2].x, r[3].x));
        st4(q + LDK, make_float4(r[0].y, r[1].y, r[2].y, r[3].y));
        st4(q + 2 * LDK, make_float4(r[0].z, r[1].z, r[2].z, r[3].z));
        st4(q + 3 * LDK, make_float4(r[0].w, r[1].w, r[2].w, r[3].w));
    }
}

struct Frags { float4 a[NG][2], b[NG][2]; };
struct Planes;
template <int SPLIT>
__device__ __forceinline__ void read_frags(Frags& f, const float* __restrict__ As, const float* __restrict__ Bs, int g) {
    const int ko = SPLIT ? 16 * (g >> 1) + 4 * (g & 1) : 8 * g;
#pragma unroll
    for (int t = 0; t < 2; ++t) {
        f.a[g][t] = ld4(As + 32 * t * LDK + ko);
        f.b[g][t] = ld4(Bs + 32 * t * LDK + ko);
    }
}
__device__ __forceinline__ void read_a(Frags& f, const float* __restrict__ As, int g) {
#pragma unroll
    for (int t = 0; t < 2; ++t) f.a[g][t] = ld4(As + 32 * t * LDK + 16 * (g >> 1) + 4 * (g & 1));
}
__device__ __forceinline__ void read_b(Frags& f, const float* __restrict__ Bs, int g) {
#pragma unroll
    for (int t = 0; t < 2; ++t) f.b[g][t] = ld4(Bs + 32 * t * LDK + 16 * (g >> 1) + 4 * (g & 1));
}
template <int SPLIT>
__device__ __forceinline__ void quarter(f32x16 (&acc)[2][2], const Frags& f, Planes (&pl)[2], int q);
__device__ __forceinline__ void mfma_group(f32x16 (&acc)[2][2], const Frags& f, int g) {
#pragma unroll
    for (int a = 0; a < 2; ++a)
#pragma unroll
        for (int b = 0; b < 2; ++b) {
            acc[a][b] = __builtin_amdgcn_mfma_f32_32x32x2f32(f.a[g][a].x, f.b[g][b].x, acc[a][b], 0, 0, 0);
            acc[a][b] = __builtin_amdgcn_mfma_f32_32x32x2f32(f.a[g][a].y, f.b[g][b].y, acc[a][b], 0, 0, 0);
            acc[a][b] = __builtin_amdgcn_mfma_f32_32x32x2f32(f.a[g][a].z, f.b[g][b].z, acc[a][b], 0, 0, 0);
            acc[a][b] = __builtin_amdgcn_mfma_f32_32x32x2f32(f.a[g][a].w, f.b[g][b].w, acc[a][b], 0, 0, 0);
        }
}
typedef __bf16 bf16x8 __attribute__((ext_vector_type(8)));
struct Planes { bf16x8 a[3][2], b[3][2]; };

__device__ __forceinline__ void split8(const float4& lo, const float4& hi, bf16x8& p1, bf16x8& p2, bf16x8& p3) {
#ifdef GEMM_AB_NOSPLIT
    p1 = __builtin_bit_cast(bf16x8, lo); p2 = __builtin_bit_cast(bf16x8, hi); p3 = p1;
    return;
#endif
    const float x[8] = {lo.x, lo.y, lo.z, lo.w, hi.x, hi.y, hi.z, hi.w};
    uint32_t w1[4], w2[4], w3[4];
// ... 304 lines not shown
    for (; i + 12 < p.nsl; i += 16) {
        const float4 u0 = ld4(s + (int64_t)i * TILE), u1 = ld4(s + (int64_t)(i + 4) * TILE);
        const float4 u2 = ld4(s + (int64_t)(i + 8) * TILE), u3 = ld4(s + (int64_t)(i + 12) * TILE);
        v.x = (((v.x + u0.x) + u1.x) + u2.x) + u3.x; v.y = (((v.y + u0.y) + u1.y) + u2.y) + u3.y;
        v.z = (((v.z + u0.z) + u1.z) + u2.z) + u3.z; v.w = (((v.w + u0.w) + u1.w) + u2.w) + u3.w;
    }
    for (; i < p.nsl; i += 4) {
        const float4 u = ld4(s + (int64_t)i * TILE);
        v.x += u.x; v.y += u.y; v.z += u.z; v.w += u.w;
    }
    if (q) part[q - 1][threadIdx.x] = v;
    __syncthreads();
    if (q) return;
    const float4 g1 = part[0][threadIdx.x], g2 = part[1][threadIdx.x], g3 = part[2][threadIdx.x];
    float o[4] = {(v.x + g1.x) + (g2.x + g3.x), (v.y + g1.y) + (g2.y + g3.y), (v.z + g1.z) + (g2.z + g3.z), (v.w + g1.w) + (g2.w + g3.w)};
    int z, m0, n0;
    tile_origin(p, p.nfull + tr, z, m0, n0);
    const int m = m0 + ml, n = n0 + nl;
    float cmax = 0.f;
    if (m < p.M && n < p.N) {
        float* c = p.C + (int64_t)z * p.sC + (int64_t)m * p.ldc + n;
#pragma unroll
        for (int j = 0; j < 4; ++j) {
            if (n + j >= p.N) break;
            float x = o[j] + (p.bias ? p.bias[(int64_t)z * p.sBias + n + j] : 0.f);
            if (p.act == 1) x = elu1(x);
            if (p.act == 3) x = softplus_nb(x);
            if (p.act == 2) x += c[j];
            c[j] = x;
            cmax = fmaxf(cmax, __builtin_fabsf(x));
        }
    }
    amax_publish_wave(cmax, p.amaxC);
}

struct Plan { int nfull, nsplit, nsl, kslice; };
constexpr int g_split_min_ksteps = 4;
inline Plan make_plan(int M, int N, int K, int batch) {
    const long nbt = (long)((M + BM - 1) / BM) * ((N + BN - 1) / BN) * batch;
    const int ksteps = (K + BK - 1) / BK;
    Plan pl{(int)nbt, 0, 1, ksteps * BK};
    const int r = (int)(nbt % GRID);
    if (r == 0 || r > GRID / 2 || ksteps < g_split_min_ksteps) return pl;
    int s = std::min(GRID / r, ksteps / 2);
    const int per = (ksteps + s - 1) / s;
    s = (ksteps + per - 1) / per;
    if (s < 2) return pl;
    pl.nfull = (int)(nbt - r); pl.nsplit = r; pl.nsl = s; pl.kslice = per * BK;
    return pl;
}

}

#ifdef GEMM_STAMP
extern "C" int resel_gemm_debug_stamps(unsigned long long* host_out) {
    return (int)hipMemcpyFromSymbol(host_out, HIP_SYMBOL(g_gemm_stamps), sizeof(unsigned long long) * 64 * 16);
}
#endif

extern "C" size_t resel_gemm_f32_workspace_bytes(int M, int N, int K, int batch) {
    if (M <= 0 || N <= 0 || K <= 0 || batch <= 0) return 0;
    const Plan pl = make_plan(M, N, K, batch);
    return std::max(std::max((size_t)pl.nsplit * pl.nsl * TILE * sizeof(float), gemm_bf3_workspace_bytes(M, N, K, batch)),
                    gemm_any_workspace_bytes(M, N, K, batch));
}

extern "C" int resel_gemm_f32(const float* A, int64_t lda, int64_t strideA, int a_kcontig,
                              const float* B, int64_t ldb, int64_t strideB, int b_kcontig,
                              const float* bias, int64_t strideBias, int act,
                              float* C, int64_t ldc, int64_t strideC, void* workspace,
                              int M, int N, int K, int batch, int split, resel_stream_t stream) {
    if (split == 2) return RESEL_EINVAL;
    return resel_gemm_f32x(A, lda, strideA, a_kcontig, B, ldb, strideB, b_kcontig, bias, strideBias, act, C, ldc, strideC, workspace,
                           M, N, K, batch, split, nullptr, nullptr, nullptr, 0u, stream);
}

extern "C" int resel_gemm_f32x(const float* A, int64_t lda, int64_t strideA, int a_kcontig,
                               const float* B, int64_t ldb, int64_t strideB, int b_kcontig,
                               const float* bias, int64_t strideBias, int act,
                               float* C, int64_t ldc, int64_t strideC, void* workspace,
                               int M, int N, int K, int batch, int split, const float* amax_a, const float* amax_b,
                               void* amax_c, unsigned amax_epoch, resel_stream_t stream) {
    if (!A || !B || !C || M <= 0 || N <= 0 || K <= 0 || batch <= 0 || act < 0 || act > 3) return RESEL_EINVAL;
    if (split != 0 && split != 2 && split != 3 && split != 6) return RESEL_EINVAL;
    if (split == 2 && (!amax_a || !amax_b)) return RESEL_EINVAL;
    if (amax_c && (reinterpret_cast<uintptr_t>(amax_c) & 7u)) return RESEL_EINVAL;
    if (split == 2 && M <= 128) split = 6;
    if (K < BK) split = 0;
    if (lda <= 0 || ldb <= 0 || ldc <= 0) return RESEL_EINVAL;
    const bool mfma_ok = !(lda % 4 || ldb % 4 || strideA % 4 || strideB % 4 || !aligned16(A) || !aligned16(B) || (a_kcontig ? K : M) % 4 ||
                           (b_kcontig ? K : N) % 4 || lda >= (int64_t)1 << 22 || ldb >= (int64_t)1 << 22);
    if (!mfma_ok || gemm_any_rows_ok(A, lda, strideA, a_kcontig, 0, B, ldb, strideB, b_kcontig, M, K, act))
        return gemm_any_launch(A, lda, strideA, a_kcontig, B, ldb, strideB, b_kcontig, bias, strideBias, act, C, ldc, strideC, workspace, M, N, K,
                               batch, 0, (unsigned long long*)amax_c, amax_epoch, (hipStream_t)stream);
    if ((split == 2 || split == 3 || split == 6) && M > 128)
        return gemm_bf3_launch(A, lda, strideA, a_kcontig, B, ldb, strideB, b_kcontig, bias, strideBias, act, C, ldc, strideC, workspace,
                               M, N, K, batch, split, (hipStream_t)stream, amax_a, amax_b, (unsigned long long*)amax_c, amax_epoch);
    if (split == 3) split = 6;
    const Plan pl = make_plan(M, N, K, batch);
    if (pl.nsplit && (!workspace || !aligned16(workspace))) return RESEL_EINVAL;
    GemmParams p{A, B, bias, C, (float*)workspace, lda, ldb, ldc, strideA, strideB, strideC, strideBias, M, N, K, act,
                 (M + BM - 1) / BM, (N + BN - 1) / BN, pl.nfull, pl.nsplit, pl.nsl, pl.kslice, AmaxOut{(unsigned long long*)amax_c, amax_epoch}};
    const int64_t total = (int64_t)pl.nfull + (int64_t)pl.nsplit * pl.nsl;
    dim3 grid((unsigned)std::min<int64_t>(total, GRID));
    hipStream_t s = (hipStream_t)stream;
#define RESEL_GEMM_LAUNCH(SP) \
    do { if (a_kcontig && b_kcontig) launch_timed(RESEL_PROF_GEMM, gemm_f32_kernel<true, true, SP>, grid, dim3(256), 0, s, p); \
         else if (a_kcontig) launch_timed(RESEL_PROF_GEMM, gemm_f32_kernel<true, false, SP>, grid, dim3(256), 0, s, p); \
         else if (b_kcontig) launch_timed(RESEL_PROF_GEMM, gemm_f32_kernel<false, true, SP>, grid, dim3(256), 0, s, p); \
         else launch_timed(RESEL_PROF_GEMM, gemm_f32_kernel<false, false, SP>, grid, dim3(256), 0, s, p); } while (0)
    if (split == 6) RESEL_GEMM_LAUNCH(6);
    else RESEL_GEMM_LAUNCH(0);
#undef RESEL_GEMM_LAUNCH
    if (pl.nsplit) hipLaunchKernelGGL(gemm_fixup_kernel, dim3(TILE / 4 / 64, pl.nsplit), dim3(64, 4), 0, s, p);
    return launch_status();
}

namespace {
__global__ __launch_bounds__(256) void head_fold_kernel(const float* __restrict__ part, int parts, int M, const float* __restrict__ b3, float* __restrict__ q) {
    const int z = blockIdx.y;
    const int m = blockIdx.x * 256 + threadIdx.x;
    if (m >= M) return;
    const float* pz = part + (int64_t)z * parts * M + m;
    float acc = b3 ? b3[z] : 0.f;
    for (int j = 0; j < parts; ++j) acc += pz[(int64_t)j * M];
    q[(int64_t)z * M + m] = acc;
}
bool fused_args_ok(const float* A, int64_t lda, int64_t strideA, int a_kcontig, const float* B, int64_t ldb, int64_t strideB, int b_kcontig,
                   const float* C, int64_t ldc, int M, int N, int K, int batch, const float* amax_a, const float* amax_b, const void* amax_c,
                   const void* workspace) {
    if (!A || !B || !C || M <= 0 || N <= 0 || K <= 0 || batch <= 0 || !amax_a || !amax_b || !workspace || !aligned16(workspace)) return false;
    if (amax_c && (reinterpret_cast<uintptr_t>(amax_c) & 7u)) return false;
    if (lda % 4 || ldb % 4 || ldc % 4 || strideA % 4 || strideB % 4 || !aligned16(A) || !aligned16(B) || !aligned16(C)) return false;
    if ((a_kcontig ? K : M) % 4 || (b_kcontig ? K : N) % 4 || N % 4) return false;
    if (lda <= 0 || ldb <= 0 || ldc <= 0) return false;
    return gemm_bf3_fused_ok(M, N, K, lda, ldb);
}
}

extern "C" int resel_gemm_f32_fused_supported(int kind, int M, int N, int K, int64_t lda, int64_t ldb) {
    if (kind == 4) return (M >= 256 && N % 128 == 0 && gemm_bf3_fused_ok(M, N, K, lda, ldb)) ? 1 : 0;
    if (kind == 5) return gemm_bf3_fused_ok(M, N, K, lda, ldb) ? 1 : 0;
    return 0;
}

extern "C" size_t resel_gemm_f32_fused_workspace_bytes(int M, int N, int K, int batch, int kind) {
    if (M <= 0 || N <= 0 || K <= 0 || batch <= 0) return 0;
    const size_t mt = M / 256, nt = (N + 127) / 128;
    const size_t own = (kind == 5 ? 2 * nt * (size_t)M : (2 * mt + 1) * (size_t)N) * batch * sizeof(float);
    return own + (kind == 4 && M % 256 ? resel_gemm_f32_workspace_bytes(M % 256, N, K, batch) + 256 : 0);
}

namespace {
__global__ __launch_bounds__(256) void dact_tail_kernel(float* __restrict__ C, int64_t ldc, int64_t sC, const float* __restrict__ Y, int64_t ldy, int64_t sY,
                                                        int rows, int N, float* __restrict__ part, int64_t part_stride, AmaxOut amax) {
    __shared__ float s_sum[4][64];
    const int c = blockIdx.x * 64 + (threadIdx.x & 63), rg = threadIdx.x >> 6, z = blockIdx.y;
    float acc = 0.f, mx = 0.f;
    if (c < N) {
        float* Cz = C + (int64_t)z * sC + c;
        const float* Yz = Y + (int64_t)z * sY + c;
        for (int r = rg; r < rows; r += 4) {
            const float y = Yz[(int64_t)r * ldy];
            const float v = Cz[(int64_t)r * ldc] * (y > 0.f ? 1.f : y + 1.f);
            Cz[(int64_t)r * ldc] = v;
            acc += v;
            mx = fmaxf(mx, __builtin_fabsf(v));
        }
    }
    s_sum[rg][threadIdx.x & 63] = acc;
    __syncthreads();
    if (rg == 0 && c < N && part) part[(int64_t)z * part_stride + c] = (s_sum[0][threadIdx.x] + s_sum[1][threadIdx.x]) + (s_sum[2][threadIdx.x] + s_sum[3][threadIdx.x]);
    amax_publish_wave(mx, amax);
}
}

extern "C" int resel_gemm_f32_dact(const float* A, int64_t lda, int64_t strideA, int a_kcontig,
                                   const float* B, int64_t ldb, int64_t strideB, int b_kcontig,
                                   const float* Y, int64_t ldy, int64_t strideY,
                                   float* C, int64_t ldc, int64_t strideC, float* dbias, void* workspace,
                                   int M, int N, int K, int batch, const float* amax_a, const float* amax_b,
                                   void* amax_c, unsigned amax_epoch, resel_stream_t stream) {
    if (!fused_args_ok(A, lda, strideA, a_kcontig, B, ldb, strideB, b_kcontig, C, ldc, M, N, K, batch, amax_a, amax_b, amax_c, workspace)) return RESEL_EINVAL;
    if (!Y || ldy % 4 || strideY % 4 || ldy <= 0 || !aligned16(Y) || !a_kcontig || M < 256 || N % 128) return RESEL_EINVAL;
    hipStream_t s = (hipStream_t)stream;
    const int Mm = M / 256 * 256, tail = M - Mm, rows = 2 * (Mm / 256) + (tail ? 1 : 0);
    float* part = dbias ? (float*)workspace : nullptr;
    int rc = gemm_bf3_launch(A, lda, strideA, a_kcontig, B, ldb, strideB, b_kcontig, nullptr, 0, 4, C, ldc, strideC, nullptr, Mm, N, K, batch, 2,
                             s, amax_a, amax_b, (unsigned long long*)amax_c, amax_epoch, Y, ldy, strideY, part, rows);
    if (rc != RESEL_OK) return rc;
    if (tail) {
        char* ws2 = (char*)workspace + ((size_t)rows * N * batch * sizeof(float) + 255) / 256 * 256;
        rc = resel_gemm_f32x(A + (int64_t)Mm * lda, lda, strideA, 1, B, ldb, strideB, b_kcontig, nullptr, 0, 0, C + (int64_t)Mm * ldc, ldc, strideC, ws2,
                             tail, N, K, batch, 2, amax_a, amax_b, nullptr, 0u, stream);
        if (rc != RESEL_OK) return rc;
        hipLaunchKernelGGL(dact_tail_kernel, dim3((N + 63) / 64, batch), dim3(256), 0, s, C + (int64_t)Mm * ldc, ldc, strideC, Y + (int64_t)Mm * ldy, ldy, strideY,
                           tail, N, part ? part + (int64_t)(rows - 1) * N : nullptr, (int64_t)rows * N, AmaxOut{(unsigned long long*)amax_c, amax_epoch});
    }
    if (dbias) launch_colsum(part, N, rows, N, dbias, s, 1, 0, batch);
    return launch_status();
}

extern "C" int resel_gemm_f32_head(const float* A, int64_t lda, int64_t strideA, int a_kcontig,
                                   const float* B, int64_t ldb, int64_t strideB, int b_kcontig,
                                   const float* bias, int64_t strideBias, const float* w3, int64_t strideW3, const float* b3,
                                   float* C, int64_t ldc, int64_t strideC, float* q, void* workspace,
                                   int M, int N, int K, int batch, const float* amax_a, const float* amax_b,
                                   void* amax_c, unsigned amax_epoch, resel_stream_t stream) {
    if (!fused_args_ok(A, lda, strideA, a_kcontig, B, ldb, strideB, b_kcontig, C, ldc, M, N, K, batch, amax_a, amax_b, amax_c, workspace)) return RESEL_EINVAL;
    if (!w3 || !q || strideW3 % 4 || !aligned16(w3)) return RESEL_EINVAL;
    const int rc = gemm_bf3_launch(A, lda, strideA, a_kcontig, B, ldb, strideB, b_kcontig, bias, strideBias, 5, C, ldc, strideC, nullptr, M, N, K, batch, 2,
                                   (hipStream_t)stream, amax_a, amax_b, (unsigned long long*)amax_c, amax_epoch, w3, 0, strideW3, (float*)workspace);
    if (rc != RESEL_OK) return rc;
    hipLaunchKernelGGL(head_fold_kernel, dim3((M + 255) / 256, batch), dim3(256), 0, (hipStream_t)stream, (const float*)workspace,
                       2 * ((N + 127) / 128), M, b3, q);
    return launch_status();
}
```

recurrent-offpolicy-rl_amd/csrc/misc.hip:

```cpp
#include "resel_common.h"
#include <cstdint>

extern "C" int resel_abi_version(void) { return 8; }

namespace { const unsigned long long* g_drop_base = nullptr; }
namespace resel { const unsigned long long* dropout_offset_base() { return g_drop_base; } }
extern "C" int resel_dropout_offset_base(const void* base) {
    if (base && ((uintptr_t)base & 7)) return RESEL_EINVAL;
    g_drop_base = (const unsigned long long*)base;
    return RESEL_OK;
}
extern "C" const char* resel_build_info(void) { return "resel_hip gfx950 (CDNA4, wave64) built " __DATE__ " " __TIME__; }

#include <utility>
#include <vector>
namespace resel {
namespace {
bool g_prof_enabled = false;
std::vector<std::pair<hipEvent_t, hipEvent_t>> g_prof_ev[RESEL_PROF_NSLOTS];
}
bool prof_on() { return g_prof_enabled; }
void prof_push(int slot, hipEvent_t a, hipEvent_t b) {
    if (slot >= 0 && slot < RESEL_PROF_NSLOTS) g_prof_ev[slot].emplace_back(a, b);
}
}

extern "C" int resel_profile_enable(int on) {
    resel::g_prof_enabled = on != 0;
    return RESEL_OK;
}

extern "C" int resel_profile_collect(int kernel_id, double* total_us, int* launches) {
    if (kernel_id < 0 || kernel_id >= RESEL_PROF_NSLOTS || !total_us || !launches) return RESEL_EINVAL;
    double tot = 0.0;
    int n = 0;
    for (auto& pr : resel::g_prof_ev[kernel_id]) {
        float ms = 0.f;
        if (hipEventSynchronize(pr.second) == hipSuccess && hipEventElapsedTime(&ms, pr.first, pr.second) == hipSuccess) {
            tot += 1e3 * ms;
            ++n;
        }
        (void)hipEventDestroy(pr.first);
        (void)hipEventDestroy(pr.second);
    }
    resel::g_prof_ev[kernel_id].clear();
    *total_us = tot;
    *launches = n;
    return RESEL_OK;
}

namespace {
struct PlaceBlock { const float* src; long long ld; int r0, nr, c0, nc; };
struct PlaceArgs { PlaceBlock b[8]; int n; };
__global__ __launch_bounds__(256) void place_blocks_kernel(float* __restrict__ out, long long ld_out, long long total, int cols, PlaceArgs a) {
    const long long i = (long long)blockIdx.x * 256 + threadIdx.x;
    if (i >= total) return;
    const int r = (int)(i / cols), c = (int)(i - (long long)r * cols);
    float v = 0.f;
#pragma unroll
    for (int k = 0; k < 8; ++k) {
        if (k < a.n) {
            const int rr = r - a.b[k].r0, cc = c - a.b[k].c0;
            if ((unsigned)rr < (unsigned)a.b[k].nr && (unsigned)cc < (unsigned)a.b[k].nc) v = a.b[k].src[(long long)rr * a.b[k].ld + cc];
        }
    }
    out[(long long)r * ld_out + c] = v;
}
}

extern "C" int resel_place_blocks(float* out, int64_t ld_out, int rows, int cols, int nblk, const float* const* src, const int64_t* ld_src,
                                  const int* r0, const int* nr, const int* c0, const int* nc, resel_stream_t stream) {
    if (!out || rows <= 0 || cols <= 0 || ld_out < cols || nblk < 0 || nblk > 8 || (nblk && (!src || !ld_src || !r0 || !nr || !c0 || !nc))) return RESEL_EINVAL;
    PlaceArgs a{};
    a.n = nblk;
    for (int k = 0; k < nblk; ++k) {
        if (!src[k] || nr[k] <= 0 || nc[k] <= 0 || r0[k] < 0 || c0[k] < 0 || r0[k] + nr[k] > rows || c0[k] + nc[k] > cols || ld_src[k] < nc[k]) return RESEL_EINVAL;
        a.b[k] = PlaceBlock{src[k], (long long)ld_src[k], r0[k], nr[k], c0[k], nc[k]};
    }
    const long long total = (long long)rows * cols;
    hipLaunchKernelGGL(place_blocks_kernel, dim3((unsigned)((total + 255) / 256)), dim3(256), 0, (hipStream_t)stream, out, (long long)ld_out, total, cols, a);
    return resel::launch_status();
}
```

recurrent-offpolicy-rl_amd/offpolicy_rnn/hip/_lib.py:

```python
import ctypes
import os
from ctypes import c_float, c_int, c_int64, c_size_t, c_uint64, c_void_p

_HERE = os.path.dirname(os.path.abspath(__file__))
LIB_PATH = os.environ.get('RESEL_HIP_LIBRARY') or os.path.join(_HERE, 'libresel_hip.so')
ABI_VERSION = 8
_lib = None

P, I, L, F, S, U = c_void_p, c_int, c_int64, c_float, c_void_p, c_uint64
E = ctypes.c_uint

SIGNATURES = {
    'resel_abi_version': (c_int, []),
    'resel_build_info': (ctypes.c_char_p, []),
    'resel_profile_enable': (c_int, [I]),
    'resel_profile_collect': (c_int, [I, P, P]),
    'resel_selective_scan_ckpt_bytes': (c_size_t, [I, I, I, I]),
    'resel_selective_scan_fwd_workspace_bytes': (c_size_t, [I, I, I, I, I]),
    'resel_selective_scan_fwd': (c_int, [P, L, P, L, P, L, P, P, L, P, L, P, P, P, P, L, P, P, P, I, I, I, I, I, I, P, E, S]),
    'resel_selective_scan_bwd_workspace_bytes': (c_size_t, [I, I, I, I, I]),
    'resel_selective_scan_bwd': (c_int, [P, L, P, L, P, L, P, P, L, P, L, P, P, P, P, L, P,
                                         P, L, P, L, P, L, P, L, P, L, P, P, P, P, I, I, I, I, I, I, P, P, E, S]),
    'resel_causal_conv1d_fwd': (c_int, [P, L, P, P, P, P, L, I, I, I, I, I, P, E, S]),
    'resel_causal_conv1d_bwd_workspace_bytes': (c_size_t, [I, I, I, I]),
    'resel_causal_conv1d_bwd': (c_int, [P, L, P, P, P, P, L, P, L, P, P, P, I, I, I, I, I, P, E, S]),
    'resel_causal_conv1d_bwd2': (c_int, [P, L, P, P, P, P, L, P, L, P, L, P, P, P, I, I, I, I, I, P, E, S]),
    'resel_add_layernorm_fwd': (c_int, [P, P, P, P, P, P, P, I, I, F, I, I, P, E, S]),
    'resel_add_layernorm_bwd_workspace_bytes': (c_size_t, [I, I]),
    'resel_add_layernorm_bwd': (c_int, [P, P, P, P, P, P, P, P, P, P, I, I, I, I, I, P, E, S]),
    'resel_linrec_real_fwd': (c_int, [P, P, L, P, P, P, I, I, I, I, P, E, S]),
    'resel_linrec_real_bwd': (c_int, [P, P, L, P, P, P, P, P, P, L, I, I, I, I, P, E, S]),
    'resel_linrec_complex_fwd': (c_int, [P, P, L, P, P, P, P, P, P, P, P, I, I, I, P, E, S]),
    'resel_linrec_complex_bwd_workspace_bytes': (c_size_t, [I, I, I]),
    'resel_place_blocks': (c_int, [P, L, I, I, I, P, P, P, P, P, P, S]),
    'resel_lru_params_fwd': (c_int, [P, P, I, S]),
    'resel_lru_params_bwd': (c_int, [P, P, P, I, S]),
    'resel_linrec_complex_bwd': (c_int, [P, P, L, P, P, P, P, P, P, P, P, P, P, P, P, L, P, P, P, P, I, I, I, S]),
    'resel_gru_workspace_bytes': (c_size_t, [I, I, I]),
    'resel_gru_seq_fwd': (c_int, [P, P, P, P, P, P, P, I, I, I, S]),
    'resel_gru_seq_bwd': (c_int, [P, P, P, P, P, P, P, P, I, I, I, S]),
    'resel_attn_varlen_fwd_workspace_bytes': (c_size_t, [I, I]),
    'resel_attn_varlen_fwd': (c_int, [P, P, P, P, P, P, I, I, I, I, I, F, F, U, U, S]),
    'resel_attn_varlen_bwd_workspace_bytes': (c_size_t, [I, I, I, I, I]),
    'resel_attn_varlen_bwd': (c_int, [P, P, P, P, P, P, P, P, I, I, I, I, I, F, F, U, U, S]),
    'resel_dropout': (c_int, [P, P, L, F, U, U, S]),
    'resel_dropout_offset_base': (c_int, [P]),
    'resel_gelu_dropout_fwd': (c_int, [P, P, L, F, U, U, P, E, S]),
    'resel_gelu_dropout_bwd': (c_int, [P, P, P, L, F, U, U, P, E, S]),
    'resel_tanh_gaussian_fwd': (c_int, [P, P, P, P, P, I, I, S]),
    'resel_tanh_gaussian_bwd': (c_int, [P, P, P, P, P, I, I, S]),
    'resel_sac_target': (c_int, [P, P, I, P, P, P, P, P, F, P, P, P, P, I, I, S]),
    'resel_sac_target_phase': (c_int, [I, P, P, I, P, P, P, P, P, F, P, P, P, P, P, I, I, S]),
    'resel_masked_loss_workspace_bytes': (c_size_t, []),
    'resel_q_loss_fwd': (c_int, [P, P, P, P, P, I, I, S]),
    'resel_q_loss_bwd': (c_int, [P, P, P, P, P, I, I, S]),
    'resel_actor_loss_fwd': (c_int, [P, P, P, P, P, P, I, I, I, I, S]),
    'resel_actor_loss_bwd': (c_int, [P, P, P, P, P, P, I, I, I, I, S]),
    'resel_sac_target_local': (c_int, [P, P, I, P, P, P, P, P, F, P, P, P, P, P, I, I, S]),
    'resel_guard_apply_slots': (c_int, [P, I, P, S]),
    'resel_sac_target_workspace_bytes': (c_size_t, [I]),
    'resel_soft_update': (c_int, [P, P, F, L, S]),
    'resel_adamw_flat': (c_int, [P, P, P, P, L, P, P, P, I, F, F, F, I, P, S]),
    'resel_adamw_flat_dev': (c_int, [P, P, P, P, L, P, P, P, I, F, F, F, P, P, S]),
    'resel_sumsq_workspace_bytes': (c_size_t, [L]),
    'resel_sumsq': (c_int, [P, L, P, P, S]),
    'resel_bias_act_fwd': (c_int, [P, P, L, I, L, I, S]),
    'resel_bias_act_bwd_workspace_bytes': (c_size_t, [L, I, L]),
    'resel_bias_act_bwd': (c_int, [P, L, P, L, P, P, P, L, I, L, I, P, E, S]),
    'resel_ensemble_head_fwd': (c_int, [P, P, P, P, P, L, I, L, S]),
    'resel_ensemble_head_bwd_workspace_bytes': (c_size_t, [L, I, L]),
    'resel_ensemble_head_bwd': (c_int, [P, P, P, P, P, P, P, L, I, L, P, E, S]),
    'resel_gemm_f32_workspace_bytes': (c_size_t, [I, I, I, I]),
    'resel_gemm_f32': (c_int, [P, L, L, I, P, L, L, I, P, L, I, P, L, L, P, I, I, I, I, I, S]),
    'resel_gemm_f32x': (c_int, [P, L, L, I, P, L, L, I, P, L, I, P, L, L, P, I, I, I, I, I, P, P, P, E, S]),
    'resel_amax_segments': (c_int, [P, P, P, I, P, E, S]),
    'resel_amax_state_bytes': (c_size_t, []),
    'resel_amax': (c_int, [P, L, L, I, I, I, P, E, P, S]),
    'resel_gemm_f32_fused_supported': (c_int, [I, I, I, I, L, L]),
    'resel_gemm_f32_fused_workspace_bytes': (c_size_t, [I, I, I, I, I]),
    'resel_gemm_f32_dact': (c_int, [P, L, L, I, P, L, L, I, P, L, L, P, L, L, P, P, I, I, I, I, P, P, P, E, S]),
    'resel_gemm_f32_head': (c_int, [P, L, L, I, P, L, L, I, P, L, P, L, P, P, L, L, P, P, I, I, I, I, P, P, P, E, S]),
    'resel_amax_check': (c_int, [P, L, L, I, I, I, P, P, I, S]),
    'resel_gemm_bf16_workspace_bytes': (c_size_t, [I, I, I]),
    'resel_gemm_bf16': (c_int, [P, L, I, I, P, L, I, I, P, P, L, I, P, I, I, I, S]),
    'resel_colsum_bf16_workspace_bytes': (c_size_t, [I, I]),
    'resel_colsum_bf16': (c_int, [P, L, I, I, P, P, S]),
    'resel_gather_trajs': (c_int, [P, I, L, P, I, I, I, I, I, I, I, I, I, P, I, P, S]),
    'resel_mamba_conv_step': (c_int, [P, L, P, L, P, L, L, L, I, P, P, P, I, I, I, I, S]),
    'resel_selective_state_update': (c_int, [P, L, P, L, P, P, L, P, P, P, P, P, L, P, I, I, I, I, S]),
    'resel_atb_workspace_bytes': (c_size_t, [L, I, I]),
    'resel_atb': (c_int, [P, L, I, P, L, I, P, I, P, L, S]),
    'resel_attn_decode': (c_int, [P, L, P, P, I, P, P, F, I, I, I, I, S]),
}


class ReselHipUnavailable(RuntimeError):
    pass


def lib():
    global _lib
    if _lib is not None:
        return _lib
    if not os.path.exists(LIB_PATH):
        raise ReselHipUnavailable(
            f'RESeL-HIP: {LIB_PATH} not found. The MI355X kernels are the only implementation of the hot path; '
            f'build them with `python -c "import __graft_entry__ as g; g.build()"` (or `make -C recurrent-offpolicy-rl_amd/csrc`).')
    handle = ctypes.CDLL(LIB_PATH)
    for name, (res, args) in SIGNATURES.items():
        fn = getattr(handle, name, None)
        if fn is None:
            raise ReselHipUnavailable(f'RESeL-HIP: symbol {name} missing from {LIB_PATH} (stale build?)')
        fn.restype = res
        fn.argtypes = args
    if handle.resel_abi_version() != ABI_VERSION:
        raise ReselHipUnavailable(f'RESeL-HIP: ABI {handle.resel_abi_version()} != expected {ABI_VERSION}; rebuild the library')
    _lib = handle
    return _lib


def check(rc: int, what: str):
    if rc != 0:
        raise RuntimeError(f'RESeL-HIP: {what} failed with code {rc} '
                           f'({ {-1: "RESEL_EINVAL (shape/alignment/null)", -2: "RESEL_ELAUNCH"}.get(rc, "?")})')
```

recurrent-offpolicy-rl_amd/offpolicy_rnn/hip/ops.py:

```python
import ctypes
import os
from typing import Optional

import torch

from ._lib import check, lib


def _need_cuda(name, *ts):
    for t in ts:
        if t is not None and not t.is_cuda:
            raise RuntimeError(f'RESeL-HIP: {name} needs CUDA tensors (got a {t.device} tensor); the HIP kernels are the '
                               f'only implementation of this op - there is no CPU fallback.')


def _p(t: Optional[torch.Tensor]):
    return None if t is None else ctypes.c_void_p(t.data_ptr())


if hasattr(torch._C, '_cuda_getCurrentRawStream') and hasattr(torch._C, '_cuda_getDevice'):
    def _stream():
        return ctypes.c_void_p(torch._C._cuda_getCurrentRawStream(torch._C._cuda_getDevice()))
else:
    def _stream():
# ... 1363 lines not shown
    check(lib().resel_amax(_p(x), x.stride(-2), x.stride(0) if x.dim() == 3 and batch > 1 else 0, x.shape[-2], x.shape[-1], batch,
                           _p(out), epoch, None, _stream()), 'amax')
    return out


def amax_value(handle):
    w = handle.view(torch.int64).cpu()[::16][:8]
    ep = (w >> 32) & 0xffffffff
    lo = (w[ep == ep.max()] & 0xffffffff).to(torch.int32)
    return float(lo.view(torch.float32).max())


PARAM_EPOCH = [0]


@torch.no_grad()
def amax_segments(flat, begin, length, handles):
    _need_cuda('amax_segments', flat, begin, length, handles)
    _AMAX_EPOCH[0] += 1
    check(lib().resel_amax_segments(_p(flat), _p(begin), _p(length), int(begin.numel()), _p(handles), _AMAX_EPOCH[0], _stream()), 'amax_segments')


def weight_amax(p):
    ref = getattr(p, '_resel_store', None)
    if ref is None or not amax_tracking():
        return None
    return ref[0].amax_handle(ref[1], p)


def _slot_args(want, device):
    if not want:
        return None, None, 0
    slot, epoch = amax_slot(device)
    return slot, _p(slot), epoch


def amax_tracking():
    return gemm_split() == 2


@torch.no_grad()
def gemm_f32(A, B, a_kcontig=True, b_kcontig=True, bias=None, act=None, out=None, split=None, amax_a=None, amax_b=None, amax_out=None):
    _need_cuda('gemm_f32', A, B)
    batched = A.dim() == 3
    assert A.stride(-1) == 1 and B.stride(-1) == 1 and A.dtype == torch.float32 and B.dtype == torch.float32
    sa_, sb_ = A.shape, B.shape
    batch = sa_[0] if batched else 1
    M, K = (sa_[-2], sa_[-1]) if a_kcontig else (sa_[-1], sa_[-2])
    N = sb_[-2] if b_kcontig else sb_[-1]
    assert (sb_[-1] if b_kcontig else sb_[-2]) == K and (not batched or sb_[0] == batch)
    if out is None:
        out = torch.empty((batch, M, N) if batched else (M, N), dtype=torch.float32, device=A.device)
    assert out.stride(-1) == 1
    GEMM_FLOPS[0] += 2.0 * M * N * K * batch
    L = lib()
    key = (M, N, K, batch)
    nb = _GEMM_WS_BYTES.get(key)
    if nb is None:
        nb = _GEMM_WS_BYTES[key] = L.resel_gemm_f32_workspace_bytes(M, N, K, batch)
    ws = _ws(nb, A.device) if nb else None
    bs = 0
    if bias is not None:
        bias = bias.reshape(batch, N) if batched else bias.reshape(N)
        bs = bias.stride(0) if batched else 0
    multi = batch > 1
    split = gemm_split() if split is None else int(split)
    global LAST_AMAX
    ha = hb = None
    if split == 2:
        if K < 32 or M <= 128:
            split = 6
        else:
            ha = amax_a if amax_a is not None else amax_of(A)
            hb = amax_b if amax_b is not None else amax_of(B)
            ha = weight_amax(A) if ha is None else ha
            hb = weight_amax(B) if hb is None else hb
            if ha is None or hb is None:
                t_gemm = 2.0 * M * N * K * batch / 1.5e8
                cost = (0.0 if ha is not None else 4.0 * M * K * batch / 4.5e6 + 2.5) + (0.0 if hb is not None else 4.0 * N * K * batch / 4.5e6 + 2.5)
                if cost <= AMAX_PREPASS_FRACTION * t_gemm:
                    if ha is None:
                        ha = amax(A)
                        tag_amax(A, ha)
                    if hb is None:
                        hb = amax(B)
                        tag_amax(B, hb)
                else:
                    split = 6
    if AMAX_VERIFY and split == 2:
        amax_check(A, ha, f'A of gemm M={M} N={N} K={K} batch={batch}')
        amax_check(B, hb, f'B of gemm M={M} N={N} K={K} batch={batch}')
    slot, slot_p, epoch = amax_out if amax_out is not None else \
        _slot_args(amax_tracking() and act != GEMM_ACCUMULATE and M * N * batch >= (1 << 20), A.device)
    check(L.resel_gemm_f32x(_p(A), A.stride(-2), A.stride(0) if multi else 0, int(a_kcontig), _p(B), B.stride(-2),
                            B.stride(0) if multi else 0, int(b_kcontig), _p(bias), bs, 2 if act == GEMM_ACCUMULATE else 3 if act == GEMM_SOFTPLUS else ACT_IDS[act], _p(out), out.stride(-2),
                            out.stride(0) if multi else 0, _p(ws), M, N, K, batch, split, _p(ha) if split == 2 else None,
                            _p(hb) if split == 2 else None, slot_p, epoch, _stream()), 'gemm_f32')
    tag_amax(out, slot)
    LAST_AMAX = slot
    LAST_SPLIT[0] = split
    return out


def _forced_handles(A, B, amax_a, amax_b):
    ha = amax_a if amax_a is not None else amax_of(A)
    hb = amax_b if amax_b is not None else amax_of(B)
    ha = weight_amax(A) if ha is None else ha
    hb = weight_amax(B) if hb is None else hb
    if ha is None:
        ha = amax(A)
        tag_amax(A, ha)
    if hb is None:
        hb = amax(B)
        tag_amax(B, hb)
    return ha, hb


def gemm_fused_ok(kind, M, N, K, *mats):
    if os.environ.get('RESEL_GEMM_FUSED', '1') == '0' or gemm_split() != 2 or not gemm_f32_ok(M, *mats) or not rows_aligned16(*mats):
        return False
    ld = max(int(t.stride(-2)) for t in mats)
    return bool(lib().resel_gemm_f32_fused_supported(int(kind), int(M), int(N), int(K), ld, ld))


@torch.no_grad()
def gemm_f32_dact(A, B, b_kcontig, Y, out, need_dbias=True, amax_a=None, amax_b=None):
    _need_cuda('gemm_f32_dact', A, B, Y, out)
    batched = A.dim() == 3
    batch = A.shape[0] if batched else 1
    M, K = A.shape[-2], A.shape[-1]
    N = B.shape[-2] if b_kcontig else B.shape[-1]
    assert (B.shape[-1] if b_kcontig else B.shape[-2]) == K and Y.shape[-2:] == (M, N) and out.shape[-2:] == (M, N)
    assert A.stride(-1) == 1 and B.stride(-1) == 1 and Y.stride(-1) == 1 and out.stride(-1) == 1
    ha, hb = _forced_handles(A, B, amax_a, amax_b)
    if AMAX_VERIFY:
        amax_check(A, ha, f'A of gemm_dact M={M} N={N} K={K} batch={batch}')
        amax_check(B, hb, f'B of gemm_dact M={M} N={N} K={K} batch={batch}')
    GEMM_FLOPS[0] += 2.0 * M * N * K * batch
    L = lib()
    ws = _ws(L.resel_gemm_f32_fused_workspace_bytes(M, N, K, batch, 4), A.device)
    dbias = torch.empty(batch, N, dtype=torch.float32, device=A.device) if need_dbias else None
    multi = batched and batch > 1
    slot, slot_p, epoch = _slot_args(amax_tracking() and M * N * batch >= (1 << 20), A.device)
    check(L.resel_gemm_f32_dact(_p(A), A.stride(-2), A.stride(0) if multi else 0, 1, _p(B), B.stride(-2), B.stride(0) if multi else 0, int(b_kcontig),
                                _p(Y), Y.stride(-2), Y.stride(0) if multi else 0, _p(out), out.stride(-2), out.stride(0) if multi else 0,
                                _p(dbias), _p(ws), M, N, K, batch, _p(ha), _p(hb), slot_p, epoch, _stream()), 'gemm_f32_dact')
    tag_amax(out, slot)
    global LAST_AMAX
    LAST_AMAX = slot
    LAST_SPLIT[0] = 2
    return out, dbias


@torch.no_grad()
def gemm_f32_head(A, B, b_kcontig, bias, w3, b3, amax_a=None, amax_b=None):
    _need_cuda('gemm_f32_head', A, B, bias, w3)
    batch, M, K = A.shape
    N = B.shape[-2] if b_kcontig else B.shape[-1]
    assert A.stride(-1) == 1 and B.stride(-1) == 1 and w3.shape == (batch, N) and w3.is_contiguous() and bias.shape == (batch, N) and bias.stride(-1) == 1
    ha, hb = _forced_handles(A, B, amax_a, amax_b)
    if AMAX_VERIFY:
        amax_check(A, ha, f'A of gemm_head M={M} N={N} K={K} batch={batch}')
        amax_check(B, hb, f'B of gemm_head M={M} N={N} K={K} batch={batch}')
    GEMM_FLOPS[0] += 2.0 * M * N * K * batch
    L = lib()
    ws = _ws(L.resel_gemm_f32_fused_workspace_bytes(M, N, K, batch, 5), A.device)
    a = torch.empty(batch, M, N, dtype=torch.float32, device=A.device)
    q = torch.empty(batch, M, dtype=torch.float32, device=A.device)
    multi = batch > 1
    slot, slot_p, epoch = _slot_args(amax_tracking() and M * N * batch >= (1 << 20), A.device)
    check(L.resel_gemm_f32_head(_p(A), A.stride(-2), A.stride(0) if multi else 0, 1, _p(B), B.stride(-2), B.stride(0) if multi else 0, int(b_kcontig),
                                _p(bias), bias.stride(0) if multi else 0, _p(w3), N, _p(b3), _p(a), a.stride(-2), a.stride(0) if multi else 0, _p(q), _p(ws),
                                M, N, K, batch, _p(ha), _p(hb), slot_p, epoch, _stream()), 'gemm_f32_head')
    tag_amax(a, slot)
    global LAST_AMAX
    LAST_AMAX = slot
    LAST_SPLIT[0] = 2
    return a, q


@torch.no_grad()
def conv_step(x, window, weight, bias, d_conv, layout, act):
    _need_cuda('conv_step', x, window)
    B, Di, K = x.shape[0], x.shape[1], d_conv
    W, sd, sk = (K, K, 1) if layout == 'dk' else (K - 1, 1, Di)
    assert window.shape == (B, Di * W) and window.stride(1) == 1 and x.stride(1) == 1
    new = torch.empty((B, Di * W), dtype=torch.float32, device=x.device)
    xc = torch.empty((B, Di), dtype=torch.float32, device=x.device)
    check(lib().resel_mamba_conv_step(_p(x), x.stride(0), _p(window), window.stride(0), _p(new), new.stride(0), sd, sk, W,
                                      _p(weight), _p(bias), _p(xc), B, Di, K, int(bool(act)), _stream()), 'mamba_conv_step')
    return xc, new


@torch.no_grad()
def selective_state_update(state, xc, x_db, dt_w, dt_b, A_log, D, z=None):
    _need_cuda('selective_state_update', state, xc, x_db)
    B, Di = xc.shape
    R = dt_w.shape[1]
    N = (x_db.shape[1] - R) // 2
    assert state.shape == (B, Di * N) and state.stride(1) == 1 and x_db.stride(1) == 1 and xc.is_contiguous()
    new = torch.empty((B, Di * N), dtype=torch.float32, device=xc.device)
    y = torch.empty_like(xc)
    check(lib().resel_selective_state_update(_p(state), state.stride(0), _p(new), new.stride(0), _p(xc), _p(x_db), x_db.stride(0),
                                             _p(dt_w), _p(dt_b), _p(A_log), _p(D), _p(z), 0 if z is None else z.stride(0), _p(y),
                                             B, Di, N, R, _stream()), 'selective_state_update')
    return y, new


@torch.no_grad()
def mamba_step(hidden, xz, conv_w, conv_b, xproj_w, dt_w, dt_b, A_log, D, d_conv, d_state):
    Di, K = xz.shape[1] // 2, d_conv
    xc, window = conv_step(xz[:, :Di], hidden[:, :Di * K], conv_w, conv_b, K, 'dk', True)
    x_db = gemm_f32(xc, xproj_w, True, True)
    y, state = selective_state_update(hidden[:, Di * K:], xc, x_db, dt_w, dt_b, A_log, D, xz[:, Di:])
    return y, torch.cat((window, state), dim=-1)


@torch.no_grad()
def attn_decode(qkv, kv_cache, pos, slopes, scale):
    _need_cuda('attn_decode', qkv, kv_cache)
    B, _, H, hd = qkv.shape
    assert qkv.dtype == torch.bfloat16 and kv_cache.dtype == torch.bfloat16 and qkv.is_contiguous() and kv_cache.is_contiguous()
    assert kv_cache.shape[0] >= B and kv_cache.shape[2:] == (2, H, hd)
    out = torch.empty((B, H, hd), dtype=torch.bfloat16, device=qkv.device)
    dev = pos if torch.is_tensor(pos) else None
    check(lib().resel_attn_decode(_p(qkv), 3 * H * hd, _p(kv_cache), _p(dev), 0 if dev is not None else int(pos), _p(slopes), _p(out),
                                  float(scale), B, H, hd, kv_cache.shape[1], _stream()), 'attn_decode')
    return out


@torch.no_grad()
def soft_update_(target_flat, online_flat, tau):
    _need_cuda('soft_update', target_flat, online_flat)
    PARAM_EPOCH[0] += 1
    check(lib().resel_soft_update(_p(target_flat), _p(online_flat), float(tau), target_flat.numel(), _stream()), 'soft_update')


@torch.no_grad()
def adamw_flat_(p, g, m, v, seg_end, seg_lr, seg_wd, step, beta1=0.9, beta2=0.999, eps=1e-8, grad_scale=None):
    _need_cuda('adamw_flat', p, g, m, v, seg_end, seg_lr, seg_wd)
    PARAM_EPOCH[0] += 1
    check(lib().resel_adamw_flat(_p(p), _p(g), _p(m), _p(v), p.numel(), _p(seg_end), _p(seg_lr), _p(seg_wd), int(seg_end.numel()),
                                 float(beta1), float(beta2), float(eps), int(step), _p(grad_scale), _stream()), 'adamw_flat')


@torch.no_grad()
def adamw_flat_dev_(p, g, m, v, seg_end, seg_lr, seg_wd, bias_corrections, beta1=0.9, beta2=0.999, eps=1e-8, grad_scale=None):
    _need_cuda('adamw_flat_dev', p, g, m, v, seg_end, seg_lr, seg_wd, bias_corrections)
    PARAM_EPOCH[0] += 1
    check(lib().resel_adamw_flat_dev(_p(p), _p(g), _p(m), _p(v), p.numel(), _p(seg_end), _p(seg_lr), _p(seg_wd), int(seg_end.numel()),
                                     float(beta1), float(beta2), float(eps), _p(bias_corrections), _p(grad_scale), _stream()), 'adamw_flat_dev')


@torch.no_grad()
def sumsq(x, out=None):
    _need_cuda('sumsq', x)
    out = torch.empty(1, dtype=torch.float32, device=x.device) if out is None else out
    ws = _ws(lib().resel_sumsq_workspace_bytes(x.numel()), x.device)
    check(lib().resel_sumsq(_p(x), x.numel(), _p(out), _p(ws), _stream()), 'sumsq')
    return out
```

recurrent-offpolicy-rl_amd/offpolicy_rnn/models/ensemble_linear_model.py:

```python
import torch
import torch.nn as nn

from ..hip import ops


def _unit(t):
    return t if t.stride(-1) == 1 else t.contiguous()


class _SharedInput(torch.autograd.Function):

    @staticmethod
    def forward(ctx, x2, weight, bias, act, x_part=None, col0=0, ax=None):
        E, n_in, n_out = weight.shape
        w_cat = weight.permute(1, 0, 2).reshape(n_in, E * n_out)
        ops.LAST_AMAX = None
        x2 = x2 if x2.stride(-1) == 1 else x2.contiguous()
        y2 = ops.gemm_f32(x2, w_cat, True, False, None if bias is None else bias.reshape(E * n_out), act, amax_a=ax,
                          amax_b=ops.weight_amax(weight))
        ax = ax if ax is not None else ops.amax_of(x2)
        ctx.save_for_backward(x2, w_cat, y2 if act is not None else None)
        ctx.ax = ops.keep_handles(ax)[0]
        ctx.dims = (E, n_in, n_out, bias is not None, act)
        ctx.part = None if x_part is None else (col0, x_part.shape[-1], tuple(x_part.shape))
        return y2.view(-1, E, n_out).transpose(0, 1)

    @staticmethod
    def backward(ctx, g):
        x2, w_cat, y2 = ctx.saved_tensors
        E, n_in, n_out, has_bias, act = ctx.dims
        g2 = g.transpose(0, 1).reshape(-1, E * n_out)
        need_db = has_bias and ctx.needs_input_grad[2]
        if act is not None:
            g2, db = ops.bias_act_bwd(g2, y2, g2.shape[0], act, need_db)
        else:
            db = g2.sum(dim=0, keepdim=True) if need_db else None
        g2 = g2 if g2.stride(-1) == 1 else g2.contiguous()
        dx = None
        if ctx.needs_input_grad[0]:
            dx = ops.gemm_f32(g2, w_cat, True, True)
        dw = None
        if ctx.needs_input_grad[1]:
            dw = ops.gemm_f32(x2, g2, False, False, amax_a=ops.handle_alive(ctx.ax))
            dw = dw.view(n_in, E, n_out).permute(1, 0, 2)
        dpart = None
        if ctx.part is not None and ctx.needs_input_grad[4]:
            col0, k, shape = ctx.part
            wp = w_cat[col0:col0 + k]
            dpart = ops.gemm_f32(g2, wp, True, True).view(shape)
        return dx, dw, None if db is None else db.view(E, 1, n_out), None, dpart, None, None


def _member_wgrad(x3, gy, ax=None):
    return ops.gemm_f32(_unit(x3), _unit(gy), False, False, amax_a=ax)


def _member_dgrad(gy, weight, like):
    E, M, _ = gy.shape
    n_in = weight.shape[1]
    if like.stride(0) < like.stride(1):
        dx = torch.empty(M, E, n_in, dtype=gy.dtype, device=gy.device).transpose(0, 1)
    else:
        dx = torch.empty(E, M, n_in, dtype=gy.dtype, device=gy.device)
    return ops.gemm_f32(_unit(gy), weight, True, True, out=dx)


class _PerMember(torch.autograd.Function):
    @staticmethod
    def forward(ctx, x3, weight, bias, act, ax=None):
        E, M, _ = x3.shape
        ops.LAST_AMAX = None
        x3 = _unit(x3)
        y = ops.gemm_f32(x3, weight, True, False, bias, act, amax_a=ax)
        ax = ax if ax is not None else ops.amax_of(x3)
        ctx.save_for_backward(x3, weight, y if act is not None else None)
        ctx.ax = ops.keep_handles(ax)[0]
        ctx.cfg = (bias is not None, act)
        return y

    @staticmethod
    def backward(ctx, g):
        x3, weight, y = ctx.saved_tensors
        has_bias, act = ctx.cfg
        E, M, n_out = g.shape
        need_db = has_bias and ctx.needs_input_grad[2]
        if act is not None or (need_db and n_out % 4 == 0):
            gy, db = ops.bias_act_bwd(g.reshape(E * M, n_out), None if y is None else y.view(E * M, n_out), M, act, need_db)
            gy = gy.view(E, M, n_out)
            db = None if db is None else db.view(E, 1, n_out)
        else:
            gy, db = g, (g.sum(dim=1, keepdim=True) if need_db else None)
        dx = _member_dgrad(gy, weight, x3) if ctx.needs_input_grad[0] else None
        dw = _member_wgrad(x3, gy, ops.handle_alive(ctx.ax)) if ctx.needs_input_grad[1] else None
        return dx, dw, db, None, None


class _Head(torch.autograd.Function):

    @staticmethod
    def forward(ctx, x3, w2, b2, w3, b3, ax=None):
        E, M, _ = x3.shape
        H = w2.shape[2]
        x3 = _unit(x3)
        a = ops.gemm_f32(x3, w2, True, False, amax_a=ax)
        ax = ax if ax is not None else ops.amax_of(x3)
        ctx.ax = ops.keep_handles(ax)[0]
        w3v = w3.reshape(E, H)
        q = ops.ensemble_head_fwd_(a, b2.reshape(E, H), w3v, None if b3 is None else b3.reshape(E))
        ctx.save_for_backward(x3, w2, w3v, a)
        ctx.has_b3 = b3 is not None
        return q.view(E, M, 1)

    @staticmethod
    def backward(ctx, gq):
        x3, w2, w3v, a = ctx.saved_tensors
        E, M, H = a.shape
        gq2 = gq.reshape(E, M)
        gy, db2, dw3 = ops.ensemble_head_bwd(gq2, a, w3v)
        dx = _member_dgrad(gy, w2, x3) if ctx.needs_input_grad[0] else None
        dw2 = _member_wgrad(x3, gy, ops.handle_alive(ctx.ax))
        db3 = gq2.sum(dim=1).view(E, 1, 1) if ctx.has_b3 else None
        return dx, dw2, db2.view(E, 1, H), dw3.view(E, H, 1), db3, None


class _CriticMLP(torch.autograd.Function):

    @staticmethod
    def forward(ctx, x2, W1, b1, W2, b2, W3, b3, x_part, col0, ax):
        E, n_in, H1 = W1.shape
        H2 = W2.shape[2]
        M = x2.shape[0]
        w_cat = W1.permute(1, 0, 2).reshape(n_in, E * H1)
        y2 = ops.gemm_f32(x2, w_cat, True, False, b1.reshape(E * H1), 'elu', amax_a=ax, amax_b=ops.weight_amax(W1))
        h_x = ax if ax is not None else ops.amax_of(x2)
        h_a1 = ops.amax_of(y2)
        a1 = y2.view(M, E, H1).transpose(0, 1)
        w3v = W3.reshape(E, H2)
        a2, q = ops.gemm_f32_head(a1, W2, False, b2.reshape(E, H2), w3v, None if b3 is None else b3.reshape(E), amax_a=h_a1,
                                  amax_b=ops.weight_amax(W2))
        ctx.save_for_backward(x2, w_cat, y2, W2, w3v, a2)
        ctx.handles = ops.keep_handles(h_x, h_a1)
        ctx.dims = (E, n_in, H1, H2, M, b3 is not None)
        ctx.part = None if x_part is None else (col0, x_part.shape[-1], tuple(x_part.shape))
        return q.view(E, M, 1)

    @staticmethod
    def backward(ctx, gq):
        x2, w_cat, y2, W2, w3v, a2 = ctx.saved_tensors
        E, n_in, H1, H2, M, has_b3 = ctx.dims
        h_x, h_a1 = ops.live_handles(ctx.handles)
        need = ctx.needs_input_grad
        gq2 = gq.reshape(E, M)
        gy2, db2, dw3 = ops.ensemble_head_bwd(gq2, a2, w3v)
        a1 = y2.view(M, E, H1).transpose(0, 1)
        dw2 = _member_wgrad(a1, gy2, h_a1) if need[3] else None
        db3 = gq2.sum(dim=1).view(E, 1, 1) if (has_b3 and need[6]) else None
        g1 = torch.empty(M, E, H1, dtype=torch.float32, device=x2.device).transpose(0, 1)
        _, db1 = ops.gemm_f32_dact(gy2, W2, True, a1, g1, need_dbias=bool(need[2]), amax_b=ops.weight_amax(W2))
        g2 = g1.transpose(0, 1).reshape(M, E * H1)
        ops.tag_amax(g2, ops.amax_of(g1))
        dx = ops.gemm_f32(g2, w_cat, True, True) if need[0] else None
        dw1 = None
        if need[1]:
            dw1 = ops.gemm_f32(x2, g2, False, False, amax_a=h_x).view(n_in, E, H1).permute(1, 0, 2)
        dpart = None
        if ctx.part is not None and need[7]:
            col0, k, shape = ctx.part
            dpart = ops.gemm_f32(g2, w_cat[col0:col0 + k], True, True).view(shape)
        return (dx, dw1, None if db1 is None else db1.view(E, 1, H1), dw2, db2.view(E, 1, H2) if need[4] else None,
                dw3.view(E, H2, 1) if need[5] else None, db3, dpart, None, None)


def critic_mlp_fusable(l0, act0, l1, act1, l2, act2, x) -> bool:
    if not (isinstance(l0, EnsembleLinear) and isinstance(l1, EnsembleLinear) and isinstance(l2, EnsembleLinear)):
        return False
    elu = lambda a: isinstance(a, nn.ELU) and a.alpha == 1.0
    if not (elu(act0) and elu(act1) and isinstance(act2, nn.Identity) and l0.use_bias and l1.use_bias):
        return False
    E = l0.active_members()
    if l1.active_members() != E or l2.active_members() != E or x.dtype != torch.float32 or not x.is_cuda:
        return False
    n_in, H1 = l0.weight.shape[1:]
    H2 = l1.weight.shape[2]
    if l1.weight.shape[1] != H1 or l2.weight.shape[1] != H2 or l2.weight.shape[2] != 1 or x.shape[-1] != n_in:
        return False
    nd = x.dim()
    if nd >= 5 or (nd in (3, 4) and (l0.desire_ndim is None or l0.desire_ndim == nd) and x.shape[0] == E):
        return False
    if not all(l.desire_ndim is None or l.desire_ndim == nd + 1 for l in (l1, l2)):
        return False
    M = x.numel() // n_in
    x2 = x.reshape(-1, n_in)
    return (min(n_in, H1, H2) >= 32 and H1 % 32 == 0 and H2 % 32 == 0 and ops.gemm_f32_ok(M, x2) and ops.rows_aligned16(x2)
            and ops.gemm_fused_ok(5, M, H2, H1, l1.weight) and ops.gemm_fused_ok(4, M, H1, H2, l1.weight))


def critic_mlp(l0: 'EnsembleLinear', l1: 'EnsembleLinear', l2: 'EnsembleLinear', x: torch.Tensor, grad_part=None) -> torch.Tensor:
    W1, b1 = l0.active_params()
    W2, b2 = l1.active_params()
    W3, b3 = l2.active_params()
    E, n_in, _ = W1.shape
    lead = tuple(x.shape[:-1])
    ax = ops.amax_of(x)
    if grad_part is not None:
        q = _CriticMLP.apply(x.detach().reshape(-1, n_in), W1, b1, W2, b2, W3, b3, grad_part[0], grad_part[1], ax)
    else:
        q = _CriticMLP.apply(x.reshape(-1, n_in), W1, b1, W2, b2, W3, b3, None, 0, ax)
    return q.reshape((E,) + lead + (1,))


def ensemble_head(hidden: 'EnsembleLinear', out: 'EnsembleLinear', x: torch.Tensor) -> torch.Tensor:
    w2, b2 = hidden.active_params()
    w3, b3 = out.active_params()
    E, n_in, H = w2.shape
    lead = tuple(x.shape[1:-1])
    q = _Head.apply(x.reshape(E, -1, n_in), w2, b2, w3, b3, ops.amax_of(x))
    return q.reshape((E,) + lead + (1,))


def head_fusable(hidden, hidden_act, out, out_act, x) -> bool:
    return (isinstance(hidden, EnsembleLinear) and isinstance(out, EnsembleLinear) and isinstance(hidden_act, nn.ELU)
            and hidden_act.alpha == 1.0 and isinstance(out_act, nn.Identity) and hidden.use_bias
            and out.weight.shape[2] == 1 and out.weight.shape[1] == hidden.weight.shape[2] and hidden.weight.shape[2] % 4 == 0
            and x.dim() >= 3 and x.shape[0] == hidden.active_members() and x.dtype == torch.float32
            and (hidden.desire_ndim is None or hidden.desire_ndim == x.dim()))


class EnsembleLinear(nn.Module):
    def __init__(self, input_dim: int, output_dim: int, num_ensemble: int, bias: bool = True, desire_ndim: int = None):
        super().__init__()
        self.use_bias = bias
        self.desire_ndim = desire_ndim
        self.num_ensemble = num_ensemble
        self.weight = nn.Parameter(torch.zeros(num_ensemble, input_dim, output_dim))
        if bias:
            self.bias = nn.Parameter(torch.zeros(num_ensemble, 1, output_dim))
        nn.init.trunc_normal_(self.weight, std=1 / (2 * input_dim ** 0.5))
        self.member_index = None

    def active_members(self) -> int:
        return self.num_ensemble if self.member_index is None else int(self.member_index.numel())

    def active_params(self):
        b = self.bias if self.use_bias else None
        if self.member_index is None:
            return self.weight, b
        return self.weight.index_select(0, self.member_index), None if b is None else b.index_select(0, self.member_index)

    def forward(self, x: torch.Tensor, act: str = None, grad_part=None) -> torch.Tensor:
        W, b = self.active_params()
        E, n_in, n_out = W.shape
        nd = x.dim()
        shared = True
        if nd == 3:
            shared = not ((self.desire_ndim is None or self.desire_ndim == 3) and x.shape[0] == E)
        elif nd == 4:
            shared = not ((self.desire_ndim is None or self.desire_ndim == 4) and x.shape[0] == E)
        elif nd == 5:
            shared = False
        ax = ops.amax_of(x)
        if shared:
            lead = tuple(x.shape[:-1])
            if grad_part is not None:
                y = _SharedInput.apply(x.detach().reshape(-1, n_in), W, b, act, grad_part[0], grad_part[1], ax)
            else:
                y = _SharedInput.apply(x.reshape(-1, n_in), W, b, act, None, 0, ax)
        else:
            assert grad_part is None, 'grad_part is a shared-input feature'
            lead = tuple(x.shape[1:-1])
            y = _PerMember.apply(x.reshape(E, -1, n_in), W, b, act, ax)
        return ops.tag_amax(y.reshape((E,) + lead + (n_out,)), ops.LAST_AMAX, whole=True)
```

Baseline: 3.012 million env-steps/s.

## Fold critic head weight into dact GEMM when head weight grads are not needed

When the backward pass does not need gradients for the second and third critic layers (for example the actor update through frozen critics), the code pre-multiplies W2 by w3 into a folded weight. The ELU-derivative transform of a2 is applied in the GEMM operand load, and gq is applied per row in the epilogue. This removes the separate ensemble_head_bwd kernel and the gy2 intermediate. In exchange it adds a small weight-fold kernel per call and a new GEMM epilogue variant, and operand A is now fixed at a unit scale for the f16 split.

```diff
diff --git a/include/resel_hip.h b/include/resel_hip.h
--- a/include/resel_hip.h
+++ b/include/resel_hip.h
@@ -186,6 +186,15 @@
                         float* C, int64_t ldc, int64_t strideC, float* q, void* workspace,
                         int M, int N, int K, int batch, const float* amax_a, const float* amax_b,
                         void* amax_c, unsigned amax_epoch, resel_stream_t stream);
+size_t resel_gemm_f32_dact_fold_workspace_bytes(int M, int N, int K, int batch);
+int resel_gemm_f32_dact_fold(const float* A, int64_t lda, int64_t strideA, const float* rowv, int64_t strideRowv,
+                             const float* B, int64_t ldb, int64_t strideB, int b_kcontig,
+                             const float* Y, int64_t ldy, int64_t strideY,
+                             float* C, int64_t ldc, int64_t strideC, float* dbias, void* workspace,
+                             int M, int N, int K, int batch, const float* amax_b,
+                             void* amax_c, unsigned amax_epoch, resel_stream_t stream);
+int resel_head_fold_weight(const float* W, int64_t ldw, int64_t strideW, const float* w3, int64_t strideW3, float* out, int E, int R, int C,
+                           void* amax_out, unsigned amax_epoch, resel_stream_t stream);
 int resel_place_blocks(float* out, int64_t ld_out, int rows, int cols, int nblk, const float* const* src, const int64_t* ld_src,
                        const int* r0, const int* nr, const int* c0, const int* nc, resel_stream_t stream);
 
diff --git a/recurrent-offpolicy-rl_amd/csrc/bias_act.hip b/recurrent-offpolicy-rl_amd/csrc/bias_act.hip
--- a/recurrent-offpolicy-rl_amd/csrc/bias_act.hip
+++ b/recurrent-offpolicy-rl_amd/csrc/bias_act.hip
@@ -1,4 +1,5 @@
 #include "resel_common.h"
+#include <algorithm>
 
 namespace {
 using namespace resel;
@@ -125,6 +126,21 @@
     }
 }
 
+__global__ __launch_bounds__(256) void fold_weight_kernel(const float* __restrict__ W, int64_t ldw, int64_t sW, const float* __restrict__ w3, int64_t sw3,
+                                                          float* __restrict__ out, int R, int C, AmaxOut amax) {
+    const int e = blockIdx.y, c4 = C / 4;
+    float mx = 0.f;
+    for (int i = blockIdx.x * 256 + threadIdx.x; i < R * c4; i += gridDim.x * 256) {
+        const int r = i / c4, c = (i - r * c4) * 4;
+        float4 v = ld4(W + (int64_t)e * sW + (int64_t)r * ldw + c);
+        const float4 w = ld4(w3 + (int64_t)e * sw3 + c);
+        v.x *= w.x; v.y *= w.y; v.z *= w.z; v.w *= w.w;
+        st4(out + ((int64_t)e * R + r) * C + c, v);
+        mx = amax4(mx, v);
+    }
+    amax_publish_wave(mx, amax);
+}
+
 inline int row_blocks(int64_t rows_per_seg) { return (int)((rows_per_seg + BWD_ROWS - 1) / BWD_ROWS); }
 inline int block_rows(int64_t, int, int64_t) { return BWD_ROWS; }
 inline int row_blocks_of(int64_t rows_per_seg, int brows) { return (int)((rows_per_seg + brows - 1) / brows); }
@@ -194,3 +210,14 @@
     launch_colsum(dw_part, H, nrb, H, dw3, s, 1, 0, nseg);
     return launch_status();
 }
+
+extern "C" int resel_head_fold_weight(const float* W, int64_t ldw, int64_t strideW, const float* w3, int64_t strideW3, float* out, int E, int R, int C,
+                                      void* amax_out, unsigned amax_epoch, resel_stream_t stream) {
+    if (amax_out && (reinterpret_cast<uintptr_t>(amax_out) & 7u)) return RESEL_EINVAL;
+    if (!W || !w3 || !out || E <= 0 || R <= 0 || C <= 0 || C % 4 || ldw < C || ldw % 4 || strideW % 4 || strideW3 % 4) return RESEL_EINVAL;
+    if (!aligned16(W) || !aligned16(w3) || !aligned16(out)) return RESEL_EINVAL;
+    const int blocks = std::min(64, (R * (C / 4) + 255) / 256);
+    hipLaunchKernelGGL(fold_weight_kernel, dim3(blocks, E), dim3(256), 0, (hipStream_t)stream, W, ldw, strideW, w3, strideW3, out, R, C,
+                       AmaxOut{(unsigned long long*)amax_out, amax_epoch});
+    return launch_status();
+}
diff --git a/recurrent-offpolicy-rl_amd/csrc/gemm_bf3.hip b/recurrent-offpolicy-rl_amd/csrc/gemm_bf3.hip
--- a/recurrent-offpolicy-rl_amd/csrc/gemm_bf3.hip
+++ b/recurrent-offpolicy-rl_amd/csrc/gemm_bf3.hip
@@ -32,6 +32,8 @@
     int64_t ldaux, sAux;
     float* red;
     int redrows;
+    const float* rowv;
+    int64_t sRowv;
 };
 
 __device__ __forceinline__ float elu1(float x) { return x > 0.f ? x : fast_exp(x) - 1.f; }
@@ -608,6 +610,8 @@
 template <bool AKC, bool BKC, int SPLIT, int EPI = 0>
 __global__ __launch_bounds__(NTH_WS, 1) void gemm_ws_kernel(Params p) {
     extern __shared__ __attribute__((aligned(16))) char lds[];
+    constexpr int XF = EPI == 6 ? 1 : 0;
+    static_assert(XF == 0 || AKC, "the head fold exists for A [rows][K]");
     constexpr bool F16 = SPLIT == 2;
     constexpr int NP = (SPLIT == 3 || SPLIT == 2) ? 2 : 3;
     constexpr int NPB = (SPLIT == 3 || SPLIT == 2) ? 2 : 3;
@@ -616,7 +620,7 @@
     const int G = gridDim.x;
     if ((int)blockIdx.x >= total) return;
     float sa_ = 1.f, sb_ = 1.f;
-    if (F16) { sa_ = f16_scale(amax_read(p.amaxA)); sb_ = f16_scale(amax_read(p.amaxB)); }
+    if (F16) { sa_ = f16_scale(XF == 1 ? 1.f : amax_read(p.amaxA)); sb_ = f16_scale(amax_read(p.amaxB)); }
     asm volatile("" :: "v"(sa_), "v"(sb_));
 
     if (__builtin_amdgcn_readfirstlane(tid) >= 256) {
@@ -681,14 +685,20 @@
             uint32_t st_off = S * STAGE;
             asm volatile("" : "+s"(st_off));
             char* st = lds + st_off;
-            auto one = [&](auto& src, auto& regs, char* pl, f32x2_t sc, auto PLc, auto NPc, auto Fc) {
+            auto one = [&](auto& src, auto& regs, char* pl, f32x2_t sc, auto PLc, auto NPc, auto Fc, auto XTc) {
                 constexpr int PL = decltype(PLc)::value, NPP = decltype(NPc)::value, FF = decltype(Fc)::value;
+                constexpr bool XT = decltype(XTc)::value;
                 typedef std::remove_reference_t<decltype(src)> ST;
+                static_assert(!XT || ST::is_kc, "the operand transform exists in the [rows][K] layout");
                 if constexpr (ST::is_kc) {
 #pragma unroll
                     for (int i = 0; i < ST::NR; ++i) {
                         if (LOAD) asm volatile("s_waitcnt vmcnt(23)" : "+v"(regs[i]) :: "memory");
-                        const float4 v = make_float4(regs[i].x, regs[i].y, regs[i].z, regs[i].w);
+                        float4 v = make_float4(regs[i].x, regs[i].y, regs[i].z, regs[i].w);
+                        if constexpr (XT) {
+                            v.x = __builtin_amdgcn_fmed3f(v.x + 1.f, 0.f, 1.f); v.y = __builtin_amdgcn_fmed3f(v.y + 1.f, 0.f, 1.f);
+                            v.z = __builtin_amdgcn_fmed3f(v.z + 1.f, 0.f, 1.f); v.w = __builtin_amdgcn_fmed3f(v.w + 1.f, 0.f, 1.f);
+                        }
                         const P3 sp = FF == 1 ? split4_f16<true>(v, sc) : FF == 2 ? split4_f16<false>(v, sc) : split4<NPP>(v);
                         char* d = pl + src.loff[0] + 4096 * i;
                         *reinterpret_cast<uint2*>(d) = sp.p1;
@@ -711,10 +721,12 @@
             };
             using IA = std::integral_constant<int, PLA>;
             using IB = std::integral_constant<int, PLB>;
-            one(a0, ra[S][0], st, scA, IA{}, std::integral_constant<int, NP>{}, std::integral_constant<int, FA>{});
-            one(a1, ra[S][1], st, scA, IA{}, std::integral_constant<int, NP>{}, std::integral_constant<int, FA>{});
-            one(b0, rb[S][0], st + 3 * PLA, scB, IB{}, std::integral_constant<int, NPB>{}, std::integral_constant<int, FB>{});
-            one(b1, rb[S][1], st + 3 * PLA, scB, IB{}, std::integral_constant<int, NPB>{}, std::integral_constant<int, FB>{});
+            using XA = std::integral_constant<bool, XF == 1>;
+            using X0 = std::integral_constant<bool, false>;
+            one(a0, ra[S][0], st, scA, IA{}, std::integral_constant<int, NP>{}, std::integral_constant<int, FA>{}, XA{});
+            one(a1, ra[S][1], st, scA, IA{}, std::integral_constant<int, NP>{}, std::integral_constant<int, FA>{}, XA{});
+            one(b0, rb[S][0], st + 3 * PLA, scB, IB{}, std::integral_constant<int, NPB>{}, std::integral_constant<int, FB>{}, X0{});
+            one(b1, rb[S][1], st + 3 * PLA, scB, IB{}, std::integral_constant<int, NPB>{}, std::integral_constant<int, FB>{}, X0{});
             if (MODE != 1) advance();
         };
         auto landed = [&]() {
@@ -805,7 +817,7 @@
     WS_BARRIER();
     rd(f0, fa[0], fb[0]);
     int cur_st = 0;
-    constexpr bool DEFER_F0 = EPI == 4;
+    constexpr bool DEFER_F0 = EPI == 4 || EPI == 6;
     for (int c_item = blockIdx.x; c_item < total; c_item += G) {
         const Item cur = decode(p, c_item);
         if (DEFER_F0 && c_item != (int)blockIdx.x) rd(f0, fa[0] + cur_st * STAGE, fb[0] + cur_st * STAGE);
@@ -956,7 +968,7 @@
         } else {
             float* C = p.C + (int64_t)cur.z * p.sC;
             const bool full_m = cur.m0 + BM <= p.M;
-            constexpr bool DACT = EPI == 4, HEAD = EPI == 5;
+            constexpr bool DACT = EPI == 4 || EPI == 6, HEAD = EPI == 5;
             const int act = EPI ? (HEAD ? 1 : 0) : p.act;
             if constexpr (DACT) {
                 constexpr int PF = 3;
@@ -977,6 +989,15 @@
                 auto ywait = [](f32x4a& r0, f32x4a& r1, f32x4a& r2, f32x4a& r3, auto NC) {
                     asm volatile("s_waitcnt vmcnt(%4)" : "+v"(r0), "+v"(r1), "+v"(r2), "+v"(r3) : "n"(decltype(NC)::value) : "memory");
                 };
+                float g0 = 0.f, g1 = 0.f;
+                const uint32_t glane = (uint32_t)(lane * 4);
+                const float* gbase = XF == 1 ? p.rowv + (int64_t)cur.z * p.sRowv + cur.m0 + wm : nullptr;
+                auto gld = [](float& r, uint32_t off, const float* base) {
+                    asm volatile("global_load_dword %0, %1, %2" : "=v"(r) : "v"(off), "s"(base) : "memory");
+                };
+                auto gwait = [](float& r0, float& r1, auto NC) {
+                    asm volatile("s_waitcnt vmcnt(%2)" : "+v"(r0), "+v"(r1) : "n"(decltype(NC)::value) : "memory");
+                };
                 auto yload = [&](auto TC) {
                     constexpr int t = decltype(TC)::value;
                     if constexpr (t < 8) {
@@ -990,18 +1011,35 @@
                     constexpr int t = decltype(TC)::value;
                     constexpr int a = t >> 1, b = t & 1;
                     yload(std::integral_constant<int, t + PF>{});
-                    ywait(yv[t][0], yv[t][1], yv[t][2], yv[t][3], std::integral_constant<int, 4 * ((t + PF < 7 ? t + PF : 7) - t)>{});
-#pragma unroll
-                    for (int g = 0; g < 4; ++g) rdp[g * 8 * 10] = make_float4(yv[t][g].x, yv[t][g].y, yv[t][g].z, yv[t][g].w);
+                    constexpr int nw = 4 * ((t + PF < 7 ? t + PF : 7) - t);
+                    if constexpr (XF == 1 && t == 0) gwait(g0, g1, std::integral_constant<int, nw>{});
+                    ywait(yv[t][0], yv[t][1], yv[t][2], yv[t][3], std::integral_constant<int, nw>{});
+                    if constexpr (XF == 1) {
+                        int ln;
+                        asm volatile("v_mbcnt_lo_u32_b32 %0, -1, 0\n\tv_mbcnt_hi_u32_b32 %0, -1, %0" : "=v"(ln));
+                        const int sb = (ln >> 3) * 4;
+#pragma unroll
+                        for (int g = 0; g < 4; ++g) {
+                            const f32x4a y = yv[t][g];
+                            const int ad = sb + 4 * ((32 * a + 8 * g) & 63);
+                            const float r = __int_as_float(__builtin_amdgcn_ds_bpermute(ad, __float_as_int(a < 2 ? g0 : g1)));
+                            rdp[g * 8 * 10] = make_float4((y.x > 0.f ? 1.f : y.x + 1.f) * r, (y.y > 0.f ? 1.f : y.y + 1.f) * r,
+                                                          (y.z > 0.f ? 1.f : y.z + 1.f) * r, (y.w > 0.f ? 1.f : y.w + 1.f) * r);
+                        }
+                    } else {
+#pragma unroll
+                        for (int g = 0; g < 4; ++g) rdp[g * 8 * 10] = make_float4(yv[t][g].x, yv[t][g].y, yv[t][g].z, yv[t][g].w);
+                    }
 #pragma unroll
                     for (int e = 0; e < 16; ++e) {
                         const float y = wr[((e & 3) + 8 * (e >> 2)) * 40];
-                        const float v = acc[a][b][e] * (y > 0.f ? 1.f : y + 1.f);
+                        const float v = XF == 1 ? acc[a][b][e] * y : acc[a][b][e] * (y > 0.f ? 1.f : y + 1.f);
                         acc[a][b][e] = v;
                         cs[b] += v;
                         cmx = fmaxf(cmx, __builtin_fabsf(v));
                     }
                 };
+                if constexpr (XF == 1) { gld(g0, glane, gbase); gld(g1, glane, gbase + 64); }
                 yload(std::integral_constant<int, 0>{}); yload(std::integral_constant<int, 1>{}); yload(std::integral_constant<int, 2>{});
                 static_assert(PF == 3, "the prologue issues PF tiles");
                 mul(std::integral_constant<int, 0>{}); mul(std::integral_constant<int, 1>{}); mul(std::integral_constant<int, 2>{});
@@ -1539,8 +1577,10 @@
 int gemm_bf3_launch(const float* A, int64_t lda, int64_t strideA, int a_kcontig, const float* B, int64_t ldb, int64_t strideB, int b_kcontig,
                     const float* bias, int64_t strideBias, int act, float* C, int64_t ldc, int64_t strideC, void* workspace,
                     int M, int N, int K, int batch, int split, hipStream_t s, const float* amaxA, const float* amaxB,
-                    unsigned long long* amax_c, unsigned amax_epoch, const float* aux, int64_t ldaux, int64_t strideAux, float* red, int redrows) {
-    if (split == 2 && (!amaxA || !amaxB)) return RESEL_EINVAL;
+                    unsigned long long* amax_c, unsigned amax_epoch, const float* aux, int64_t ldaux, int64_t strideAux, float* red, int redrows,
+                    const float* rowv, int64_t strideRowv) {
+    if (split == 2 && (!amaxB || (!amaxA && !rowv))) return RESEL_EINVAL;
+    if (rowv && (act != 4 || !a_kcontig)) return RESEL_EINVAL;
     Plan pl = make_plan(M, N, K, batch);
     if (act >= 4) {
         if (split != 2 || !gemm_bf3_fused_ok(M, N, K, lda, ldb) || !aux) return RESEL_EINVAL;
@@ -1551,7 +1591,7 @@
     if (pl.nsplit && (!workspace || !aligned16(workspace))) return RESEL_EINVAL;
     Params p{A, B, bias, C, (float*)workspace, lda, ldb, ldc, strideA, strideB, strideC, strideBias, M, N, K, act,
              (M + BM - 1) / BM, (N + BN - 1) / BN, pl.nfull, pl.nsplit, pl.nsl, pl.kslice, amaxA, amaxB, AmaxOut{amax_c, amax_epoch}, g_nt,
-             aux, ldaux, strideAux, red, redrows};
+             aux, ldaux, strideAux, red, redrows, rowv, strideRowv};
     const int64_t total = (int64_t)pl.nfull + (int64_t)pl.nsplit * pl.nsl;
     dim3 grid((unsigned)std::min<int64_t>(total, GRID));
     int rc;
@@ -1587,7 +1627,8 @@
     }
     if (act >= 4) {
         if (!a_kcontig) return RESEL_EINVAL;
-        if (act == 4) rc = b_kcontig ? launch_ws<true, true, 2, 4>(p, grid, s) : launch_ws<true, false, 2, 4>(p, grid, s);
+        if (act == 4 && rowv) rc = b_kcontig ? launch_ws<true, true, 2, 6>(p, grid, s) : launch_ws<true, false, 2, 6>(p, grid, s);
+        else if (act == 4) rc = b_kcontig ? launch_ws<true, true, 2, 4>(p, grid, s) : launch_ws<true, false, 2, 4>(p, grid, s);
         else rc = b_kcontig ? launch_ws<true, true, 2, 5>(p, grid, s) : launch_ws<true, false, 2, 5>(p, grid, s);
     } else if (ws) WS_LAUNCH(2);
     else if (split == 3) BF3_LAUNCH(3); else if (split == 2) BF3_LAUNCH(2); else BF3_LAUNCH(6);
diff --git a/recurrent-offpolicy-rl_amd/csrc/gemm_f32.hip b/recurrent-offpolicy-rl_amd/csrc/gemm_f32.hip
--- a/recurrent-offpolicy-rl_amd/csrc/gemm_f32.hip
+++ b/recurrent-offpolicy-rl_amd/csrc/gemm_f32.hip
@@ -8,7 +8,7 @@
                     const float* bias, int64_t strideBias, int act, float* C, int64_t ldc, int64_t strideC, void* workspace,
                     int M, int N, int K, int batch, int split, hipStream_t s, const float* amaxA, const float* amaxB,
                     unsigned long long* amax_c, unsigned amax_epoch, const float* aux = nullptr, int64_t ldaux = 0, int64_t strideAux = 0,
-                    float* red = nullptr, int redrows = 0);
+                    float* red = nullptr, int redrows = 0, const float* rowv = nullptr, int64_t strideRowv = 0);
 bool gemm_bf3_fused_ok(int M, int N, int K, int64_t lda, int64_t ldb);
 }
 
@@ -619,8 +619,10 @@
 }
 
 namespace {
+template <bool ROWV = false>
 __global__ __launch_bounds__(256) void dact_tail_kernel(float* __restrict__ C, int64_t ldc, int64_t sC, const float* __restrict__ Y, int64_t ldy, int64_t sY,
-                                                        int rows, int N, float* __restrict__ part, int64_t part_stride, AmaxOut amax) {
+                                                        int rows, int N, float* __restrict__ part, int64_t part_stride, AmaxOut amax,
+                                                        const float* __restrict__ rowv = nullptr, int64_t sRowv = 0) {
     __shared__ float s_sum[4][64];
     const int c = blockIdx.x * 64 + (threadIdx.x & 63), rg = threadIdx.x >> 6, z = blockIdx.y;
     float acc = 0.f, mx = 0.f;
@@ -629,7 +631,8 @@
         const float* Yz = Y + (int64_t)z * sY + c;
         for (int r = rg; r < rows; r += 4) {
             const float y = Yz[(int64_t)r * ldy];
-            const float v = Cz[(int64_t)r * ldc] * (y > 0.f ? 1.f : y + 1.f);
+            const float d = ROWV ? (y > 0.f ? 1.f : y + 1.f) * rowv[(int64_t)z * sRowv + r] : (y > 0.f ? 1.f : y + 1.f);
+            const float v = Cz[(int64_t)r * ldc] * d;
             Cz[(int64_t)r * ldc] = v;
             acc += v;
             mx = fmaxf(mx, __builtin_fabsf(v));
@@ -661,8 +664,66 @@
         rc = resel_gemm_f32x(A + (int64_t)Mm * lda, lda, strideA, 1, B, ldb, strideB, b_kcontig, nullptr, 0, 0, C + (int64_t)Mm * ldc, ldc, strideC, ws2,
                              tail, N, K, batch, 2, amax_a, amax_b, nullptr, 0u, stream);
         if (rc != RESEL_OK) return rc;
-        hipLaunchKernelGGL(dact_tail_kernel, dim3((N + 63) / 64, batch), dim3(256), 0, s, C + (int64_t)Mm * ldc, ldc, strideC, Y + (int64_t)Mm * ldy, ldy, strideY,
+        hipLaunchKernelGGL(dact_tail_kernel<false>, dim3((N + 63) / 64, batch), dim3(256), 0, s, C + (int64_t)Mm * ldc, ldc, strideC, Y + (int64_t)Mm * ldy, ldy, strideY,
                            tail, N, part ? part + (int64_t)(rows - 1) * N : nullptr, (int64_t)rows * N, AmaxOut{(unsigned long long*)amax_c, amax_epoch});
+    }
+    if (dbias) launch_colsum(part, N, rows, N, dbias, s, 1, 0, batch);
+    return launch_status();
+}
+
+namespace {
+__global__ __launch_bounds__(256) void fold_tail_kernel(const float* __restrict__ A, int64_t lda, int64_t sA, int rows, int K, float* __restrict__ T,
+                                                        unsigned long long* one) {
+    const int z = blockIdx.y, k4 = K / 4;
+    for (int i = blockIdx.x * 256 + threadIdx.x; i < rows * k4; i += gridDim.x * 256) {
+        const int r = i / k4, k = (i - r * k4) * 4;
+        float4 v = ld4(A + (int64_t)z * sA + (int64_t)r * lda + k);
+        v.x = __builtin_amdgcn_fmed3f(v.x + 1.f, 0.f, 1.f); v.y = __builtin_amdgcn_fmed3f(v.y + 1.f, 0.f, 1.f);
+        v.z = __builtin_amdgcn_fmed3f(v.z + 1.f, 0.f, 1.f); v.w = __builtin_amdgcn_fmed3f(v.w + 1.f, 0.f, 1.f);
+        st4(T + ((int64_t)z * rows + r) * K + k, v);
+    }
+    if (blockIdx.x == 0 && z == 0 && threadIdx.x < RESEL_AMAX_SUBSLOTS) one[RESEL_AMAX_STRIDE * threadIdx.x] = __float_as_uint(1.f);
+}
+size_t fold_tail_bytes(int M, int N, int K, int batch) {
+    const int tail = M % 256;
+    if (!tail) return 0;
+    return (size_t)RESEL_AMAX_SUBSLOTS * RESEL_AMAX_STRIDE * 8 + ((size_t)tail * K * batch * sizeof(float) + 255) / 256 * 256;
+}
+}
+
+extern "C" size_t resel_gemm_f32_dact_fold_workspace_bytes(int M, int N, int K, int batch) {
+    if (M <= 0 || N <= 0 || K <= 0 || batch <= 0) return 0;
+    return resel_gemm_f32_fused_workspace_bytes(M, N, K, batch, 4) + fold_tail_bytes(M, N, K, batch);
+}
+
+extern "C" int resel_gemm_f32_dact_fold(const float* A, int64_t lda, int64_t strideA, const float* rowv, int64_t strideRowv,
+                                        const float* B, int64_t ldb, int64_t strideB, int b_kcontig,
+                                        const float* Y, int64_t ldy, int64_t strideY,
+                                        float* C, int64_t ldc, int64_t strideC, float* dbias, void* workspace,
+                                        int M, int N, int K, int batch, const float* amax_b,
+                                        void* amax_c, unsigned amax_epoch, resel_stream_t stream) {
+    if (!fused_args_ok(A, lda, strideA, 1, B, ldb, strideB, b_kcontig, C, ldc, M, N, K, batch, amax_b, amax_b, amax_c, workspace)) return RESEL_EINVAL;
+    if (!Y || ldy % 4 || strideY % 4 || ldy <= 0 || !aligned16(Y) || M < 256 || N % 128) return RESEL_EINVAL;
+    if (!rowv || strideRowv < 0 || (batch > 1 && strideRowv < M)) return RESEL_EINVAL;
+    hipStream_t s = (hipStream_t)stream;
+    const int Mm = M / 256 * 256, tail = M - Mm, rows = 2 * (Mm / 256) + (tail ? 1 : 0);
+    float* part = dbias ? (float*)workspace : nullptr;
+    int rc = gemm_bf3_launch(A, lda, strideA, 1, B, ldb, strideB, b_kcontig, nullptr, 0, 4, C, ldc, strideC, nullptr, Mm, N, K, batch, 2,
+                             s, nullptr, amax_b, (unsigned long long*)amax_c, amax_epoch, Y, ldy, strideY, part, rows, rowv, strideRowv);
+    if (rc != RESEL_OK) return rc;
+    if (tail) {
+        char* ws2 = (char*)workspace + resel_gemm_f32_fused_workspace_bytes(M, N, K, batch, 4);
+        unsigned long long* one = (unsigned long long*)ws2;
+        float* T = (float*)(ws2 + (size_t)RESEL_AMAX_SUBSLOTS * RESEL_AMAX_STRIDE * 8);
+        const int nblk = std::min(64, (tail * (K / 4) + 255) / 256);
+        hipLaunchKernelGGL(fold_tail_kernel, dim3(nblk, batch), dim3(256), 0, s, A + (int64_t)Mm * lda, lda, strideA, tail, K, T, one);
+        char* ws3 = (char*)workspace + ((size_t)rows * N * batch * sizeof(float) + 255) / 256 * 256;
+        rc = resel_gemm_f32x(T, K, (int64_t)tail * K, 1, B, ldb, strideB, b_kcontig, nullptr, 0, 0, C + (int64_t)Mm * ldc, ldc, strideC, ws3,
+                             tail, N, K, batch, 2, (const float*)one, amax_b, nullptr, 0u, stream);
+        if (rc != RESEL_OK) return rc;
+        hipLaunchKernelGGL(dact_tail_kernel<true>, dim3((N + 63) / 64, batch), dim3(256), 0, s, C + (int64_t)Mm * ldc, ldc, strideC, Y + (int64_t)Mm * ldy, ldy, strideY,
+                           tail, N, part ? part + (int64_t)(rows - 1) * N : nullptr, (int64_t)rows * N, AmaxOut{(unsigned long long*)amax_c, amax_epoch},
+                           rowv + Mm, strideRowv);
     }
     if (dbias) launch_colsum(part, N, rows, N, dbias, s, 1, 0, batch);
     return launch_status();
diff --git a/recurrent-offpolicy-rl_amd/csrc/misc.hip b/recurrent-offpolicy-rl_amd/csrc/misc.hip
--- a/recurrent-offpolicy-rl_amd/csrc/misc.hip
+++ b/recurrent-offpolicy-rl_amd/csrc/misc.hip
@@ -1,7 +1,7 @@
 #include "resel_common.h"
 #include <cstdint>
 
-extern "C" int resel_abi_version(void) { return 8; }
+extern "C" int resel_abi_version(void) { return 9; }
 
 namespace { const unsigned long long* g_drop_base = nullptr; }
 namespace resel { const unsigned long long* dropout_offset_base() { return g_drop_base; } }
diff --git a/recurrent-offpolicy-rl_amd/offpolicy_rnn/hip/_lib.py b/recurrent-offpolicy-rl_amd/offpolicy_rnn/hip/_lib.py
--- a/recurrent-offpolicy-rl_amd/offpolicy_rnn/hip/_lib.py
+++ b/recurrent-offpolicy-rl_amd/offpolicy_rnn/hip/_lib.py
@@ -4,7 +4,7 @@
 
 _HERE = os.path.dirname(os.path.abspath(__file__))
 LIB_PATH = os.environ.get('RESEL_HIP_LIBRARY') or os.path.join(_HERE, 'libresel_hip.so')
-ABI_VERSION = 8
+ABI_VERSION = 9
 _lib = None
 
 P, I, L, F, S, U = c_void_p, c_int, c_int64, c_float, c_void_p, c_uint64
@@ -79,6 +79,9 @@
     'resel_gemm_f32_fused_supported': (c_int, [I, I, I, I, L, L]),
     'resel_gemm_f32_fused_workspace_bytes': (c_size_t, [I, I, I, I, I]),
     'resel_gemm_f32_dact': (c_int, [P, L, L, I, P, L, L, I, P, L, L, P, L, L, P, P, I, I, I, I, P, P, P, E, S]),
+    'resel_gemm_f32_dact_fold_workspace_bytes': (c_size_t, [I, I, I, I]),
+    'resel_gemm_f32_dact_fold': (c_int, [P, L, L, P, L, P, L, L, I, P, L, L, P, L, L, P, P, I, I, I, I, P, P, E, S]),
+    'resel_head_fold_weight': (c_int, [P, L, L, P, L, P, I, I, I, P, E, S]),
     'resel_gemm_f32_head': (c_int, [P, L, L, I, P, L, L, I, P, L, P, L, P, P, L, L, P, P, I, I, I, I, P, P, P, E, S]),
     'resel_amax_check': (c_int, [P, L, L, I, I, I, P, P, I, S]),
     'resel_gemm_bf16_workspace_bytes': (c_size_t, [I, I, I]),
diff --git a/recurrent-offpolicy-rl_amd/offpolicy_rnn/hip/ops.py b/recurrent-offpolicy-rl_amd/offpolicy_rnn/hip/ops.py
--- a/recurrent-offpolicy-rl_amd/offpolicy_rnn/hip/ops.py
+++ b/recurrent-offpolicy-rl_amd/offpolicy_rnn/hip/ops.py
@@ -1539,6 +1539,49 @@
     return out, dbias
 
 
+def head_fold_enabled():
+    return os.environ.get('RESEL_HEAD_FOLD', '1') != '0'
+
+
+@torch.no_grad()
+def head_fold_weight(W2, w3):
+    _need_cuda('head_fold_weight', W2, w3)
+    E, R, C = W2.shape
+    assert W2.stride(-1) == 1 and w3.shape == (E, C) and w3.stride(-1) == 1
+    out = torch.empty(E, R, C, dtype=torch.float32, device=W2.device)
+    slot, epoch = amax_slot(W2.device)
+    check(lib().resel_head_fold_weight(_p(W2), W2.stride(1), W2.stride(0), _p(w3), w3.stride(0), _p(out), E, R, C, _p(slot), epoch, _stream()),
+          'head_fold_weight')
+    return out, slot
+
+
+@torch.no_grad()
+def gemm_f32_dact_fold(a2, gq, Bf, hb, Y, out, need_dbias=True):
+    _need_cuda('gemm_f32_dact_fold', a2, gq, Bf, Y, out)
+    E, M, K = a2.shape
+    N = Bf.shape[1]
+    gq = gq if gq.stride(-1) == 1 else gq.contiguous()
+    assert Bf.shape == (E, N, K) and gq.shape == (E, M) and Y.shape == (E, M, N) and out.shape == (E, M, N)
+    assert a2.stride(-1) == 1 and Bf.stride(-1) == 1 and Y.stride(-1) == 1 and out.stride(-1) == 1
+    if AMAX_VERIFY:
+        amax_check(Bf, hb, f'B of gemm_dact_fold M={M} N={N} K={K} batch={E}')
+    GEMM_FLOPS[0] += 2.0 * M * N * K * E
+    L = lib()
+    ws = _ws(L.resel_gemm_f32_dact_fold_workspace_bytes(M, N, K, E), a2.device)
+    dbias = torch.empty(E, N, dtype=torch.float32, device=a2.device) if need_dbias else None
+    multi = E > 1
+    slot, slot_p, epoch = _slot_args(amax_tracking() and M * N * E >= (1 << 20), a2.device)
+    check(L.resel_gemm_f32_dact_fold(_p(a2), a2.stride(-2), a2.stride(0) if multi else 0, _p(gq), gq.stride(0) if multi else 0,
+                                     _p(Bf), Bf.stride(-2), Bf.stride(0) if multi else 0, 1, _p(Y), Y.stride(-2), Y.stride(0) if multi else 0,
+                                     _p(out), out.stride(-2), out.stride(0) if multi else 0, _p(dbias), _p(ws), M, N, K, E, _p(hb), slot_p, epoch,
+                                     _stream()), 'gemm_f32_dact_fold')
+    tag_amax(out, slot)
+    global LAST_AMAX
+    LAST_AMAX = slot
+    LAST_SPLIT[0] = 2
+    return out, dbias
+
+
 @torch.no_grad()
 def gemm_f32_head(A, B, b_kcontig, bias, w3, b3, amax_a=None, amax_b=None):
     _need_cuda('gemm_f32_head', A, B, bias, w3)
diff --git a/recurrent-offpolicy-rl_amd/offpolicy_rnn/models/ensemble_linear_model.py b/recurrent-offpolicy-rl_amd/offpolicy_rnn/models/ensemble_linear_model.py
--- a/recurrent-offpolicy-rl_amd/offpolicy_rnn/models/ensemble_linear_model.py
+++ b/recurrent-offpolicy-rl_amd/offpolicy_rnn/models/ensemble_linear_model.py
@@ -151,12 +151,17 @@
         h_x, h_a1 = ops.live_handles(ctx.handles)
         need = ctx.needs_input_grad
         gq2 = gq.reshape(E, M)
-        gy2, db2, dw3 = ops.ensemble_head_bwd(gq2, a2, w3v)
         a1 = y2.view(M, E, H1).transpose(0, 1)
-        dw2 = _member_wgrad(a1, gy2, h_a1) if need[3] else None
         db3 = gq2.sum(dim=1).view(E, 1, 1) if (has_b3 and need[6]) else None
         g1 = torch.empty(M, E, H1, dtype=torch.float32, device=x2.device).transpose(0, 1)
-        _, db1 = ops.gemm_f32_dact(gy2, W2, True, a1, g1, need_dbias=bool(need[2]), amax_b=ops.weight_amax(W2))
+        if not (need[3] or need[4] or need[5]) and ops.head_fold_enabled():
+            wf, hwf = ops.head_fold_weight(W2, w3v)
+            _, db1 = ops.gemm_f32_dact_fold(a2, gq2, wf, hwf, a1, g1, need_dbias=bool(need[2]))
+            dw2 = db2 = dw3 = None
+        else:
+            gy2, db2, dw3 = ops.ensemble_head_bwd(gq2, a2, w3v)
+            dw2 = _member_wgrad(a1, gy2, h_a1) if need[3] else None
+            _, db1 = ops.gemm_f32_dact(gy2, W2, True, a1, g1, need_dbias=bool(need[2]), amax_b=ops.weight_amax(W2))
         g2 = g1.transpose(0, 1).reshape(M, E * H1)
         ops.tag_amax(g2, ops.amax_of(g1))
         dx = ops.gemm_f32(g2, w_cat, True, True) if need[0] else None
```

Result: no change. 3.033 million env-steps/s, median of 6 (+0.7%).
